# IONIQ6000/av1-go

Hardware: AMD Instinct MI355X
Metric: encoded 4K30 frames/sec (whole node) at fixed QP; PSNR-Y delta vs libaom (higher is better)
Workload: dtype u16

## Files before the change

av1-go_amd/av1stream.py:

```python
import ctypes as C
import os
import subprocess

import numpy as np

_HOST = os.path.join(os.path.dirname(os.path.abspath(__file__)), "host", "libav1mi_host.so")
_lib = None


class ObuFrame(C.Structure):
    _fields_ = [("width", C.c_int32), ("height", C.c_int32), ("bit_depth", C.c_int32), ("frame_type", C.c_int32),
                ("base_q_idx", C.c_int32), ("lf_level", C.c_int32 * 4), ("lf_sharpness", C.c_int32), ("cdef_damping", C.c_int32),
                ("cdef_bits", C.c_int32), ("cdef_y", C.c_uint8 * 8), ("cdef_uv", C.c_uint8 * 8), ("cdef_idx", C.c_void_p),
                ("lr_type", C.c_int32 * 3), ("lr_unit_shift", C.c_int32), ("lr_uv_shift", C.c_int32), ("lr_units", C.c_void_p * 3),
                ("reduced_tx_set", C.c_int32), ("disable_cdf_update", C.c_int32), ("tile_cols_log2", C.c_int32),
                ("tile_rows_log2", C.c_int32), ("y_mode", C.c_void_p), ("angle_y", C.c_void_p), ("uv_mode", C.c_void_p),
                ("angle_uv", C.c_void_p), ("cfl_alpha", C.c_void_p), ("skip", C.c_void_p), ("tx_type", C.c_void_p),
                ("is_inter", C.c_void_p), ("mv", C.c_void_p), ("lev_y", C.c_void_p), ("lev_u", C.c_void_p), ("lev_v", C.c_void_p),
                ("visible_width", C.c_int32), ("visible_height", C.c_int32)]


def lib():
    global _lib
    if _lib is None:
        if not os.path.exists(_HOST):
            subprocess.check_call(["make", "-s", "-C", os.path.dirname(_HOST)])
        _lib = C.CDLL(_HOST)
        _lib.av1mi_obu_write_temporal_unit.restype = C.c_longlong
        _lib.av1mi_obu_write_temporal_unit.argtypes = [C.POINTER(ObuFrame), C.c_int, C.c_int, C.c_void_p, C.c_longlong, C.c_char_p, C.c_int]
        _lib.av1mi_host_opstream_temporal_unit.restype = C.c_longlong
        _lib.av1mi_host_opstream_temporal_unit.argtypes = [C.POINTER(ObuFrame), C.c_int, C.c_void_p, C.c_longlong, C.c_char_p, C.c_int]
    return _lib


_PTR_FIELDS = {"cdef_idx": np.uint8, "y_mode": np.uint8, "angle_y": np.int8, "uv_mode": np.uint8, "angle_uv": np.int8, "cfl_alpha": np.int8,
               "skip": np.uint8, "tx_type": np.uint8, "is_inter": np.uint8, "mv": np.int16, "lev_y": np.int16, "lev_u": np.int16,
               "lev_v": np.int16}


def temporal_unit(width, height, bit_depth, base_q_idx, frame_type=0, with_sequence_header=True, threads=1, lf_level=(0, 0, 0, 0),
                  lf_sharpness=0, cdef_damping=3, cdef_bits=0, cdef_y=(0,), cdef_uv=(0,), lr_type=(0, 0, 0), lr_unit_shift=0, lr_uv_shift=0,
                  lr_units=(None, None, None), reduced_tx_set=0, disable_cdf_update=0, tile_cols_log2=-1, tile_rows_log2=-1, opstream=False,
                  visible=None, key_rows32=0, **arrays):
    f = ObuFrame()
    f.width, f.height, f.bit_depth, f.frame_type, f.base_q_idx = width, height, bit_depth, frame_type, base_q_idx
    if visible is not None:
        f.visible_width, f.visible_height = int(visible[0]), int(visible[1])
    for i in range(4):
        f.lf_level[i] = int(lf_level[i])
    f.lf_sharpness, f.cdef_damping, f.cdef_bits = lf_sharpness, cdef_damping, cdef_bits
    for i, v in enumerate(cdef_y):
        f.cdef_y[i] = int(v)
    for i, v in enumerate(cdef_uv):
        f.cdef_uv[i] = int(v)
    keep = []
    for p in range(3):
        f.lr_type[p] = int(lr_type[p])
        if lr_units[p] is not None:
            a = np.ascontiguousarray(lr_units[p], np.int8)
            keep.append(a)
            f.lr_units[p] = a.ctypes.data
    f.lr_unit_shift, f.lr_uv_shift = lr_unit_shift, lr_uv_shift
    f.reduced_tx_set, f.disable_cdf_update, f.tile_cols_log2, f.tile_rows_log2 = reduced_tx_set, disable_cdf_update, tile_cols_log2, tile_rows_log2
    for k, v in arrays.items():
        if k not in _PTR_FIELDS:
            raise TypeError("unknown field " + k)
        if v is None:
            continue
        a = np.ascontiguousarray(v, _PTR_FIELDS[k])
        keep.append(a)
        setattr(f, k, a.ctypes.data)
    cap = width * height * 4 + (1 << 16)
    out = np.empty(cap, np.uint8)
    err = C.create_string_buffer(256)
    if opstream:
        h = lib()
        h.av1mi_host_opstream_key32_temporal_unit.restype = C.c_longlong
        h.av1mi_host_opstream_key32_temporal_unit.argtypes = [C.POINTER(ObuFrame), C.c_int, C.c_int, C.c_void_p, C.c_longlong, C.c_char_p, C.c_int]
        n = h.av1mi_host_opstream_key32_temporal_unit(C.byref(f), int(key_rows32), int(with_sequence_header), out.ctypes.data, cap, err, 256)
    else:
        n = lib().av1mi_obu_write_temporal_unit(C.byref(f), int(with_sequence_header), threads, out.ctypes.data, cap, err, 256)
    if n < 0:
        raise ValueError("av1 bitstream writer: " + err.value.decode())
    if n > cap:
        raise RuntimeError("temporal unit of %d bytes exceeds the buffer" % n)
    return out[:n].tobytes()


BLOCK_DTYPE = np.dtype([("mi_row", "<u2"), ("mi_col", "<u2"), ("bsize", "u1"), ("skip", "u1"), ("is_inter", "u1"), ("y_mode", "u1"), ("uv_mode", "u1"),
                        ("angle_y", "i1"), ("angle_uv", "i1"), ("cfl_alpha_u", "i1"), ("cfl_alpha_v", "i1"), ("tx_depth", "u1"), ("interp_filter", "u1"),
                        ("reserved", "u1"), ("mv_x", "<i2"), ("mv_y", "<i2"), ("tx_type_off", "<u4"), ("lev_off", "<u4", (3,))])
assert BLOCK_DTYPE.itemsize == 36


class ObuBlocks(C.Structure):
    _fields_ = [("hdr", ObuFrame), ("tx_mode_select", C.c_int32), ("interp_filter", C.c_int32), ("high_precision_mv", C.c_int32), ("partition", C.c_void_p), ("n_partition", C.c_size_t),
                ("blocks", C.c_void_p), ("n_blocks", C.c_size_t), ("tx_type", C.c_void_p), ("levels", C.c_void_p)]


def blocks_temporal_unit(width, height, bit_depth, base_q_idx, partition, blocks, tx_type, levels, frame_type=0, with_sequence_header=True,
                         tx_mode_select=0, interp_filter=0, high_precision_mv=0, reduced_tx_set=0, disable_cdf_update=0, tile_cols_log2=-1,
                         tile_rows_log2=-1, lf_level=(0, 0, 0, 0), lf_sharpness=0, cdef_damping=3, cdef_bits=0, cdef_y=(0,), cdef_uv=(0,), cdef_idx=None,
                         lr_type=(0, 0, 0), lr_units=(None, None, None), lr_unit_shift=0, lr_uv_shift=0):
    d = ObuBlocks()
    f = d.hdr
    f.width, f.height, f.bit_depth, f.frame_type, f.base_q_idx = width, height, bit_depth, frame_type, base_q_idx
    for i in range(4):
        f.lf_level[i] = int(lf_level[i])
    f.lf_sharpness, f.cdef_damping, f.cdef_bits = lf_sharpness, cdef_damping, cdef_bits
    for i, v in enumerate(cdef_y):
        f.cdef_y[i] = int(v)
    for i, v in enumerate(cdef_uv):
        f.cdef_uv[i] = int(v)
    f.reduced_tx_set, f.disable_cdf_update, f.tile_cols_log2, f.tile_rows_log2 = reduced_tx_set, disable_cdf_update, tile_cols_log2, tile_rows_log2
    keep = [np.ascontiguousarray(partition, np.uint8), np.ascontiguousarray(blocks, BLOCK_DTYPE), np.ascontiguousarray(tx_type, np.uint8),
            np.ascontiguousarray(levels, np.int16)]
    if cdef_idx is not None:
        keep.append(np.ascontiguousarray(cdef_idx, np.uint8))
        f.cdef_idx = keep[-1].ctypes.data
    for p in range(3):
        f.lr_type[p] = int(lr_type[p])
        if lr_units[p] is not None:
            keep.append(np.ascontiguousarray(lr_units[p], np.int8))
            f.lr_units[p] = keep[-1].ctypes.data
    f.lr_unit_shift, f.lr_uv_shift = lr_unit_shift, lr_uv_shift
    d.tx_mode_select, d.interp_filter, d.high_precision_mv = int(tx_mode_select), int(interp_filter), int(high_precision_mv)
    d.partition, d.n_partition, d.blocks, d.n_blocks = keep[0].ctypes.data, keep[0].size, keep[1].ctypes.data, keep[1].size
    d.tx_type, d.levels = keep[2].ctypes.data, keep[3].ctypes.data
    cap = width * height * 4 + (1 << 16)
    out = np.empty(cap, np.uint8)
    err = C.create_string_buffer(256)
    L = lib()
    L.av1mi_obu_write_blocks_temporal_unit.restype = C.c_longlong
    L.av1mi_obu_write_blocks_temporal_unit.argtypes = [C.POINTER(ObuBlocks), C.c_int, C.c_void_p, C.c_longlong, C.c_char_p, C.c_int]
    n = L.av1mi_obu_write_blocks_temporal_unit(C.byref(d), int(with_sequence_header), out.ctypes.data, cap, err, 256)
    if n < 0:
        raise ValueError("av1 block writer: " + err.value.decode())
    if n > cap:
        raise RuntimeError("temporal unit of %d bytes exceeds the buffer" % n)
    return out[:n].tobytes()


def assemble_temporal_unit(width, height, bit_depth, base_q_idx, payloads, sizes, with_sequence_header=True, **hdr):
    f = ObuFrame()
    f.width, f.height, f.bit_depth, f.base_q_idx = width, height, bit_depth, base_q_idx
    if hdr.get("visible") is not None:
        f.visible_width, f.visible_height = int(hdr["visible"][0]), int(hdr["visible"][1])
    f.frame_type = hdr.get("frame_type", 0)
    for i in range(4):
        f.lf_level[i] = int(hdr.get("lf_level", (0,) * 4)[i])
    f.lf_sharpness, f.cdef_damping, f.cdef_bits = hdr.get("lf_sharpness", 0), hdr.get("cdef_damping", 3), 0
    f.cdef_y[0], f.cdef_uv[0] = int(hdr.get("cdef_y", (0,))[0]), int(hdr.get("cdef_uv", (0,))[0])
    keep = []
    for p in range(3):
        f.lr_type[p] = int(hdr.get("lr_type", (0, 0, 0))[p])
        u = hdr.get("lr_units", (None,) * 3)[p]
        if u is not None:
            a = np.ascontiguousarray(u, np.int8)
            keep.append(a)
            f.lr_units[p] = a.ctypes.data
    f.lr_unit_shift, f.lr_uv_shift = hdr.get("lr_unit_shift", 0), hdr.get("lr_uv_shift", 0)
    f.tile_cols_log2 = f.tile_rows_log2 = -1
    pay = np.ascontiguousarray(payloads, np.uint8)
    sz = np.ascontiguousarray(sizes, np.uint32)
    cap = int(pay.size) + (1 << 16) + 4 * int(sz.size)
    out = np.empty(cap, np.uint8)
    err = C.create_string_buffer(256)
    L = lib()
    L.av1mi_obu_assemble_temporal_unit.restype = C.c_longlong
    L.av1mi_obu_assemble_temporal_unit.argtypes = [C.POINTER(ObuFrame), C.c_void_p, C.c_void_p, C.c_int, C.c_int, C.c_void_p, C.c_longlong, C.c_char_p, C.c_int]
    n = L.av1mi_obu_assemble_temporal_unit(C.byref(f), pay.ctypes.data, sz.ctypes.data, int(sz.size), int(with_sequence_header), out.ctypes.data, cap, err, 256)
    if n < 0 or n > cap:
        raise ValueError("assemble: " + err.value.decode())
    return out[:n].tobytes()


def session_frame_unit_gpu(width, height, bit_depth, frame, seg, with_sequence_header=None, visible=None):
    p = frame["params"]
    hdr = header_from_params(p, width, height, frame["lr_on"][seg], visible)
    nt = frame["tiles_per_frame"]
    sizes = frame["tile_size"][seg * nt:(seg + 1) * nt]
    start = int(frame["tile_size"][:seg * nt].sum(dtype=np.uint64))
    pay = frame["tile_payload"][start:start + int(sizes.sum(dtype=np.uint64))]
    sh = (p.frame_type == 0) if with_sequence_header is None else with_sequence_header
    return assemble_temporal_unit(width, height, bit_depth, p.base_q_idx, pay, sizes, with_sequence_header=sh, **hdr)


def session_temporal_unit(width, height, bit_depth, raw_frame, seg, with_sequence_header=True, threads=1, visible=None):
    h = lib()
    h.av1mi_session_temporal_unit.restype = C.c_longlong
    h.av1mi_session_temporal_unit.argtypes = [C.c_void_p, C.c_int, C.c_int, C.c_int, C.c_int, C.c_int, C.c_int, C.c_int, C.c_int, C.c_void_p, C.c_longlong,
                                              C.c_char_p, C.c_int]
    cap = width * height * 4 + (1 << 16)
    out = np.empty(cap, np.uint8)
    err = C.create_string_buffer(256)
    vw, vh = visible if visible is not None else (0, 0)
    n = h.av1mi_session_temporal_unit(C.addressof(raw_frame), int(seg), width, height, bit_depth, int(vw), int(vh), int(with_sequence_header), int(threads),
                                      out.ctypes.data, cap, err, 256)
    if n < 0:
        raise ValueError("av1mi_session_temporal_unit: " + err.value.decode())
    return out[:n].tobytes()


def header_from_params(p, width, height, lr_on=None, visible=None):
    ur = lambda n: max(1, (n + p.lr_unit_size // 2) // p.lr_unit_size)
    vw, vh = visible if visible is not None else (width, height)
    uy = np.tile(np.array(list(p.lr_unit_y), np.int8), (ur(vh), ur(vw), 1))
    uc = np.tile(np.array(list(p.lr_unit_uv), np.int8), (ur((vh + 1) // 2), ur((vw + 1) // 2), 1))
    shift = {64: 0, 128: 1, 256: 2}[p.lr_unit_size]
    types = [int(p.lr_unit_y[0]), int(p.lr_unit_uv[0]), int(p.lr_unit_uv[0])]
    if lr_on is not None:
        types = [t if int(k) else 0 for t, k in zip(types, lr_on)]
    return dict(frame_type=p.frame_type, lf_level=tuple(p.lf_level), lf_sharpness=p.lf_sharpness, cdef_damping=p.cdef_damping,
                cdef_y=(p.cdef_y,), cdef_uv=(p.cdef_uv,), lr_type=tuple(types), lr_unit_shift=shift, lr_uv_shift=0, lr_units=(uy, uc, uc),
                **({} if visible is None else {"visible": (int(vw), int(vh))}))


def session_frame_unit(width, height, bit_depth, frame, seg, with_sequence_header=None, threads=1, visible=None):
    p = frame["params"]
    hdr = header_from_params(p, width, height, frame["lr_on"][seg], visible)
    if p.frame_type == 0:
        sym = dict(y_mode=frame["y_mode"][seg], uv_mode=frame["uv_mode"][seg])
    else:
        sym = dict(mv=frame["mv"][seg], skip=frame["skip"][seg])
    sh = (p.frame_type == 0) if with_sequence_header is None else with_sequence_header
    return temporal_unit(width, height, bit_depth, p.base_q_idx, with_sequence_header=sh, threads=threads, lev_y=frame["lev_y"][seg],
                         lev_u=frame["lev_u"][seg], lev_v=frame["lev_v"][seg], **sym, **hdr)
```

av1-go_amd/csrc/av1_entropy_kernels.hip:

```cpp
#include <string.h>
#include <vector>
#include "av1_ops_cdfs.hpp"
#include "av1_ops32.hpp"
#include "av1mi_internal.hpp"

namespace av1mi {
using namespace av1ops;

struct Av1EntLaunch {
  FrameView fv;
  int nframes, sbr_n, sbc_n;
  BlockInfo *info;
  op_t *ops; uint32_t ops_cap;
  uint32_t *grouped; uint32_t grouped_cap;
  uint16_t *slot_total, *slot_base;
  uint16_t *rec;
  uint32_t *nops;
  uint8_t *slots; uint32_t slot_cap;
  uint32_t *tile_size;
  uint64_t *tile_off;
  uint32_t *status;
  uint8_t *out; uint64_t out_cap;
  const uint16_t *cdf_image; int cdf_words;
  SlotTable tab;
  const uint16_t *cdf_image32; SlotTable tab32;
  const uint8_t *lr_on_frame;
  int sb_rows32, band, nslots;
};

__device__ __forceinline__ FrameView frame_view(const Av1EntLaunch &L, int f) {
  FrameView v = L.fv;
  const long nb = (long)v.w8 * v.h8;
  if (v.key) { v.y_mode += nb * f; v.uv_mode += nb * f; }
  else { v.mv += nb * 2 * f; v.skip += nb * f; }
  v.lev_y += nb * 64 * f; v.lev_u += nb * 16 * f; v.lev_v += nb * 16 * f;
  v.info = L.info + nb * f;
  if (L.lr_on_frame) for (int p = 0; p < 3; p++) v.lr_on[p] = v.lr_on[p] && L.lr_on_frame[f * 3 + p];
  return v;
}

__global__ __launch_bounds__(256) void k_av1_info(Av1EntLaunch L) {
  const long nb = (long)L.fv.w8 * L.fv.h8, i = (long)blockIdx.x * 256 + threadIdx.x;
  if (i >= nb * L.nframes) return;
  const int f = (int)(i / nb), b = (int)(i - (long)f * nb);
  const FrameView v = frame_view(L, f);
  BlockInfo o = {};
  block_summary(v, b, &o);
  if (!v.key) inter_mode_decision(v, b / v.w8, b % v.w8, &o);
  L.info[nb * f + b] = o;
}

constexpr int kReplaySlots = (S_MAX + 1) / 2;
struct TokLds {
  union {
    struct { uint8_t cnt[S_MAX * kBlocksPerTile]; alignas(16) uint8_t mag[kBlocksPerTile * kMagBytes]; } p1;
    uint16_t pos[kReplaySlots * kBlocksPerTile];
  };
  uint16_t total[S_MAX], base[S_MAX];
  ScanTables scan;
};

__global__ __launch_bounds__(64) __attribute__((amdgpu_waves_per_eu(2, 8))) void k_av1_tokens(Av1EntLaunch L) {
  const int tiles = L.sbr_n * L.sbc_n, t = blockIdx.x, f = t / tiles, tt = t - f * tiles, sbr = tt / L.sbc_n, sbc = tt - sbr * L.sbc_n;
  if (sbr < L.sb_rows32) return;
  const FrameView v = frame_view(L, f);
  const int zi = threadIdx.x, nslots = v.key ? S_KEY_END : S_INTER_END;
  __shared__ TokLds S;
  {
    uint32_t *m = reinterpret_cast<uint32_t *>(S.p1.cnt);
    for (int i = zi; i < S_MAX * kBlocksPerTile / 4; i += 64) m[i] = 0;
    if (zi == 0) fill_scan_tables(&S.scan);
  }
  __syncthreads();
  uint16_t *rec = L.rec + ((size_t)t * kBlocksPerTile + zi) * kBlockRecords;
  const TokScratch ts = { S.p1.mag + zi * kMagBytes, &S.scan };
  Sink k = { rec, S.p1.cnt, zi, 0, 0, false };
  tok_block(v, k, ts, sbr, sbc, zi);
  int x = k.n;
#pragma unroll
  for (int d = 1; d < 64; d <<= 1) {
    const int y = __shfl_up(x, d, 64);
    if (zi >= d) x += y;
  }
  const int total = __shfl(x, 63, 64), first = x - k.n;
  if ((uint32_t)total > L.ops_cap || __any(k.overflow)) {
    if (zi == 0) { atomicOr(L.status, 1u); L.nops[t] = 0; }
    for (int sl = zi; sl < S_MAX; sl += 64) L.slot_total[(size_t)t * S_MAX + sl] = 0;
    return;
  }
  if (zi == 0) L.nops[t] = (uint32_t)total;
  __syncthreads();
  constexpr int kOwn = (S_MAX + 63) / 64;
  uint32_t c[kOwn][kBlocksPerTile / 4];
#pragma unroll
  for (int q = 0; q < kOwn; q++) {
    const int sl = zi + 64 * q;
    int sum = 0;
#pragma unroll
    for (int w = 0; w < kBlocksPerTile / 4; w++) {
      const uint32_t u = sl < nslots ? reinterpret_cast<const uint32_t *>(S.p1.cnt)[sl * (kBlocksPerTile / 4) + w] : 0u;
      c[q][w] = u;
      sum = (int)__builtin_amdgcn_sad_u8(u, 0u, (unsigned)sum);
    }
    if (sl < S_MAX) S.total[sl] = (uint16_t)sum;
  }
  __syncthreads();
  {
    int mine = 0;
    for (int q = 0; q < 4; q++) { const int sl = 4 * zi + q; if (sl < nslots) mine += (S.total[sl] + kListAlign - 1) & ~(kListAlign - 1); }
    int inc = mine;
#pragma unroll
    for (int d = 1; d < 64; d <<= 1) {
      const int y = __shfl_up(inc, d, 64);
      if (zi >= d) inc += y;
    }
    int run = inc - mine;
    for (int q = 0; q < 4; q++) { const int sl = 4 * zi + q; if (sl < nslots) { S.base[sl] = (uint16_t)run; run += (S.total[sl] + kListAlign - 1) & ~(kListAlign - 1); } }
  }
  __syncthreads();
#pragma unroll
  for (int q = 0; q < kOwn; q++) {
    const int sl = zi + 64 * q;
    if (sl >= S_MAX) continue;
    const bool on = sl < nslots;
    L.slot_total[(size_t)t * S_MAX + sl] = on ? S.total[sl] : (uint16_t)0;
    L.slot_base[(size_t)t * S_MAX + sl] = on ? S.base[sl] : (uint16_t)0;
  }
  op_t *list = L.ops + (size_t)t * L.ops_cap;
  uint32_t *grouped = L.grouped + (size_t)t * L.grouped_cap;
#pragma unroll
  for (int half = 0; half < 2; half++) {
    const int lo = half * kReplaySlots, hi = lo + kReplaySlots;
    if (half) __syncthreads();
#pragma unroll
    for (int q = 0; q < kOwn; q++) {
      const int sl = zi + 64 * q;
      if (sl < lo || sl >= hi || sl >= nslots) continue;
      int run = S.base[sl];
#pragma unroll
      for (int w = 0; w < kBlocksPerTile / 4; w++) {
        const uint32_t u = c[q][w];
        const int p0 = run, p1 = p0 + (int)(u & 0xFF), p2 = p1 + (int)((u >> 8) & 0xFF), p3 = p2 + (int)((u >> 16) & 0xFF);
        run = p3 + (int)(u >> 24);
        uint32_t *d = reinterpret_cast<uint32_t *>(S.pos + (sl - lo) * kBlocksPerTile + 4 * w);
        d[0] = (uint32_t)p0 | ((uint32_t)p1 << 16); d[1] = (uint32_t)p2 | ((uint32_t)p3 << 16);
      }
    }
    __syncthreads();
    __threadfence_block();
    replay_block<kBlocksPerTile>(rec, k.nrec, S.pos, zi, first, list, grouped, lo, hi, half == 0);
  }
}

constexpr int kTiles32 = 16;
static_assert(kBlocks32 * kMag32Bytes >= K_END * kBlocks32 * 2 && kMag32Bytes % 8 == 0, "a tile's counters live where its four magnitude maps were");
__global__ __launch_bounds__(64) void k_av1_tokens32(Av1EntLaunch L, int ntiles_all) {
  __shared__ ScanTables32 scan;
  __shared__ __attribute__((aligned(16))) uint8_t s_mag[64 * kMag32Bytes];
  __shared__ Sum32 s_sum[kTiles32][kBlocks32];
  __shared__ int s_n[kTiles32][kBlocks32], s_nrec[kTiles32][kBlocks32], s_bad[kTiles32];
  const int tiles = L.sbr_n * L.sbc_n, tl = threadIdx.x >> 2, b = threadIdx.x & 3, t = blockIdx.x * kTiles32 + tl;
  bool live = t < ntiles_all;
  int f = 0, sbr = 0, sbc = 0;
  if (live) { f = t / tiles; const int tt = t - f * tiles; sbr = tt / L.sbc_n; sbc = tt - sbr * L.sbc_n; live = sbr < L.sb_rows32; }
  fill_scan_tables32(&scan, (int)threadIdx.x, 64);
  if (b == 0) s_bad[tl] = 0;
  const FrameView v = frame_view(L, live ? f : 0);
  const bool inside = live && !((b & 1) && sbc * 8 + 4 >= v.w8);
  if (inside) block_sums32(v, block_index32(v, sbr, sbc, b), &s_sum[tl][b]);
  __syncthreads();
  uint16_t *rec = L.rec + ((size_t)(live ? t : 0) * kBlocks32 + b) * kBlockRecords32;
  int nrec = 0;
  if (live) { s_n[tl][b] = 0; s_nrec[tl][b] = 0; }
  if (inside) {
    Sink32 k = { rec, nullptr, b, (int)kBlockRecords32, 0, 0, false, 0, 0, 0, 0 };
    const TokScratch32 ts = { s_mag + threadIdx.x * kMag32Bytes, &scan };
    tok_block32(v, k, ts, sbr, sbc, b, s_sum[tl]);
    s_n[tl][b] = k.n; s_nrec[tl][b] = nrec = k.nrec;
    if (k.overflow) atomicOr(&s_bad[tl], 1);
  }
  __syncthreads();
  uint16_t *cnt = reinterpret_cast<uint16_t *>(s_mag + tl * kBlocks32 * kMag32Bytes);
  for (int i = b; i < K_END * kBlocks32; i += kBlocks32) cnt[i] = 0;
  __syncthreads();
  if (live && !count_block32(rec, nrec, cnt, b)) atomicOr(&s_bad[tl], 1);
  __syncthreads();
  if (live && b == 0) {
    uint16_t *total = L.slot_total + (size_t)t * S_MAX, *base = L.slot_base + (size_t)t * S_MAX;
    const int run = place_tile32(cnt, total, base);
    for (int sl = K_END; sl < S_MAX; sl++) { total[sl] = 0; base[sl] = 0; }
    const int n = s_n[tl][0] + s_n[tl][1] + s_n[tl][2] + s_n[tl][3];
    if (s_bad[tl] || (uint32_t)n > L.ops_cap || run > 65535) {
      s_bad[tl] = 1;
      atomicOr(L.status, 1u);
      L.nops[t] = 0;
      for (int sl = 0; sl < K_END; sl++) total[sl] = 0;
    } else {
      L.nops[t] = (uint32_t)n;
    }
  }
  __syncthreads();
  if (!live || s_bad[tl]) return;
  int first = 0;
  for (int q = 0; q < b; q++) first += s_n[tl][q];
  replay_block<kBlocks32>(rec, nrec, cnt, b, first, L.ops + (size_t)t * L.ops_cap, L.grouped + (size_t)t * L.grouped_cap);
}

__global__ __launch_bounds__(64) void k_av1_chains(Av1EntLaunch L, int ntiles_all, int ngroups) {
  const int xcd = blockIdx.x & 7, j = blockIdx.x >> 3, nslots = L.nslots;
  const int g = (j / nslots) * 8 + xcd, sl = j - (j / nslots) * nslots, lane = threadIdx.x, t = g * 64 + lane;
  if (g >= ngroups) return;
  __shared__ __attribute__((aligned(16))) uint16_t s_big[64 * 16];
  const int n = L.tab.nsym[sl], off = L.tab.off[sl];
  int cnt = 0, base = 0;
  bool mine = t < ntiles_all;
  if (mine && L.band) { const int tiles = L.sbr_n * L.sbc_n, sbr = (t % tiles) / L.sbc_n; mine = (sbr < L.sb_rows32) == (L.band == 1); }
  if (mine) { cnt = L.slot_total[(size_t)t * S_MAX + sl]; base = L.slot_base[(size_t)t * S_MAX + sl]; }
  if (!__any(cnt > 0)) return;
  const size_t tt = t < ntiles_all ? (size_t)t : 0;
  op_t *list = L.ops + tt * L.ops_cap;
  const uint32_t *grouped = L.grouped + tt * L.grouped_cap + base;
  if (n <= 4) {
    const uint32_t *iw = reinterpret_cast<const uint32_t *>(L.cdf_image) + (off >> 1);
    uint64_t cdf = (uint64_t)iw[0] | ((uint64_t)iw[1] << 32);
    const uint4 *g4 = reinterpret_cast<const uint4 *>(grouped);
    const uint4 z = make_uint4(0, 0, 0, 0);
    uint4 c0 = cnt > 0 ? g4[0] : z, c1 = cnt > 4 ? g4[1] : z, c2 = cnt > 8 ? g4[2] : z, c3 = cnt > 12 ? g4[3] : z;
    auto four = [&](const uint4 &v, int e) {
      if (e < cnt) list[v.x >> 4] = small_step(cdf, (int)(v.x & 15), n);
      if (e + 1 < cnt) list[v.y >> 4] = small_step(cdf, (int)(v.y & 15), n);
      if (e + 2 < cnt) list[v.z >> 4] = small_step(cdf, (int)(v.z & 15), n);
      if (e + 3 < cnt) list[v.w >> 4] = small_step(cdf, (int)(v.w & 15), n);
    };
#pragma unroll 1
    for (int e = 0; e < cnt; e += 16) {
      const uint4 *nx = g4 + (e >> 2) + 4;
      const uint4 n0 = e + 16 < cnt ? nx[0] : z, n1 = e + 20 < cnt ? nx[1] : z, n2 = e + 24 < cnt ? nx[2] : z, n3 = e + 28 < cnt ? nx[3] : z;
      four(c0, e); four(c1, e + 4); four(c2, e + 8); four(c3, e + 12);
      c0 = n0; c1 = n1; c2 = n2; c3 = n3;
    }
  } else {
    uint16_t *cdf = s_big + lane * 16;
    {
      const uint4 *iw = reinterpret_cast<const uint4 *>(L.cdf_image + off);
      uint4 *d = reinterpret_cast<uint4 *>(cdf);
      d[0] = iw[0];
      d[1] = n > 8 ? iw[1] : make_uint4(0, 0, 0, 0);
    }
#pragma unroll 1
    for (int e = 0; e < cnt; e++) {
      const uint32_t v = grouped[e];
      const int s = (int)(v & 15);
      list[v >> 4] = s >= kSplitHorz ? split_tuple(cdf, s) : big_step(cdf, s, n);
    }
  }
}

constexpr int kRingOps = 64, kLaneWords = kRingOps * 2 + Coder::kStage + 8;

__global__ __launch_bounds__(64) void k_av1_code(Av1EntLaunch L, int ntiles_all) {
  __shared__ __attribute__((aligned(16))) uint16_t s_lane[64 * kLaneWords];
  const int lane = threadIdx.x, t = blockIdx.x * 64 + lane;
  const bool live = t < ntiles_all;
  uint32_t *ring = reinterpret_cast<uint32_t *>(s_lane + lane * kLaneWords);
  Coder c;
  c.init(L.slots + (size_t)(live ? t : 0) * L.slot_cap, (int)L.slot_cap, s_lane + lane * kLaneWords + kRingOps * 2);
  const int n = live ? (int)L.nops[t] : 0;
  const uint4 *ops4 = reinterpret_cast<const uint4 *>(L.ops + (size_t)(live ? t : 0) * L.ops_cap);
  uint4 r0, r1, r2, r3, r4, r5, r6, r7;
  r0 = r1 = r2 = r3 = r4 = r5 = r6 = r7 = make_uint4(0, 0, 0, 0);
  int w = 0;
  bool pend = false;
  auto request = [&]() {
    const uint4 *p = ops4 + (w >> 2);
    if (w < n) r0 = p[0];
    if (w + 4 < n) r1 = p[1];
    if (w + 8 < n) r2 = p[2];
    if (w + 12 < n) r3 = p[3];
    if (w + 16 < n) r4 = p[4];
    if (w + 20 < n) r5 = p[5];
    if (w + 24 < n) r6 = p[6];
    if (w + 28 < n) r7 = p[7];
    pend = w < n;
  };
  auto take = [&]() {
    uint4 *q = reinterpret_cast<uint4 *>(ring + (w & 32));
    q[0] = r0; q[1] = r1; q[2] = r2; q[3] = r3; q[4] = r4; q[5] = r5; q[6] = r6; q[7] = r7;
    w += 32;
  };
  request();
  if (pend) { take(); request(); }
  int i = 0, lit_left = 0;
  uint32_t op = ring[0], op_next = ring[1], op_next2 = ring[2];
  for (;;) {
    if (!__any(lit_left > 0 || i < n)) break;
    if (__any((pend && w - i < 24) || c.ns >= Coder::kStage - 8)) {
      if (pend && w - i <= 32) { take(); request(); }
      c.spill();
    }
#pragma unroll
    for (int q = 0; q < 8; q++) {
      if (lit_left > 0 || i < n) {
        const uint32_t fetched = ring[(i + 3) & (kRingOps - 1)];
        uint32_t tup = op;
        if (lit_left == 0 && (op >> 31)) lit_left = (int)((op >> 27) & 15);
        if (lit_left > 0) {
          lit_left--;
          tup = (op >> lit_left) & 1 ? (1u << 19) | (256u << 9) : (2u << 19) | (512u << 9) | 256u;
        }
        c.encode_tuple(tup);
        if (lit_left == 0) { i++; op = op_next; op_next = op_next2; op_next2 = fetched; }
      }
    }
  }
  if (!live) return;
  int sz = n ? c.finish() : -1;
  if (sz < 0) { if (n) atomicOr(L.status, 2u); sz = 0; }
  L.tile_size[t] = (uint32_t)sz;
}

__global__ __launch_bounds__(1024) void k_av1_scan(Av1EntLaunch L, int ntiles_all) {
  __shared__ uint64_t part[1024];
  const int tid = threadIdx.x, per = (ntiles_all + 1023) / 1024, i0 = tid * per, i1 = min(i0 + per, ntiles_all);
  uint64_t s = 0;
  for (int i = i0; i < i1; i++) s += L.tile_size[i];
  part[tid] = s;
  __syncthreads();
  for (int d = 1; d < 1024; d <<= 1) {
    const uint64_t y = tid >= d ? part[tid - d] : 0;
    __syncthreads();
    part[tid] += y;
    __syncthreads();
  }
  uint64_t run = part[tid] - s;
  for (int i = i0; i < i1; i++) { L.tile_off[i] = run; run += L.tile_size[i]; }
  if (tid == 1023) {
    L.tile_off[ntiles_all] = part[1023];
    if (part[1023] > L.out_cap) atomicOr(L.status, 4u);
  }
}
__global__ __launch_bounds__(64) void k_av1_gather(Av1EntLaunch L) {
  const int t = blockIdx.x;
  const uint32_t n = L.tile_size[t];
  const uint64_t off = L.tile_off[t];
  if (off + n > L.out_cap) return;
  const uint8_t *src = L.slots + (size_t)t * L.slot_cap;
  uint8_t *dst = L.out + off;
  const uint32_t head = min(n, (uint32_t)((16 - (reinterpret_cast<uintptr_t>(dst) & 15)) & 15)), body = (n - head) >> 4, tail0 = head + (body << 4);
  if (threadIdx.x < head) dst[threadIdx.x] = src[threadIdx.x];
  for (uint32_t i = threadIdx.x; i < body; i += 64) {
    uint4 v;
    __builtin_memcpy(&v, src + head + 16 * i, 16);
    *reinterpret_cast<uint4 *>(dst + head + 16 * i) = v;
  }
  if (tail0 + threadIdx.x < n) dst[tail0 + threadIdx.x] = src[tail0 + threadIdx.x];
}

hipError_t launch_av1_front(av1mi_ctx *ctx, const Av1EntLaunch &L, hipStream_t s) {
  const long nb = (long)L.fv.w8 * L.fv.h8 * L.nframes;
  const int ntiles_all = L.sbr_n * L.sbc_n * L.nframes, ngroups = (ntiles_all + 63) / 64;
  ProfToken t = ctx_prof_begin(ctx, AV1MI_K_ENTROPY_TOKENS, s);
  hipLaunchKernelGGL(k_av1_info, dim3((unsigned)((nb + 255) / 256)), dim3(256), 0, s, L);
  if (L.sb_rows32 < L.sbr_n) hipLaunchKernelGGL(k_av1_tokens, dim3((unsigned)ntiles_all), dim3(64), 0, s, L);
  if (L.sb_rows32) hipLaunchKernelGGL(k_av1_tokens32, dim3((unsigned)((ntiles_all + kTiles32 - 1) / kTiles32)), dim3(64), 0, s, L, ntiles_all);
  ctx_prof_end(ctx, t, s);
  t = ctx_prof_begin(ctx, AV1MI_K_ENTROPY_CHAINS, s);
  Av1EntLaunch C = L;
  C.nslots = L.fv.key ? S_KEY_END : S_INTER_END; C.band = L.sb_rows32 ? 2 : 0;
  if (L.sb_rows32 < L.sbr_n) hipLaunchKernelGGL(k_av1_chains, dim3((unsigned)(((ngroups + 7) / 8) * 8 * C.nslots)), dim3(64), 0, s, C, ntiles_all, ngroups);
  if (L.sb_rows32) {
    C.nslots = K_END; C.band = 1; C.tab = L.tab32; C.cdf_image = L.cdf_image32;
    hipLaunchKernelGGL(k_av1_chains, dim3((unsigned)(((ngroups + 7) / 8) * 8 * C.nslots)), dim3(64), 0, s, C, ntiles_all, ngroups);
  }
  ctx_prof_end(ctx, t, s);
  return hipGetLastError();
}
hipError_t launch_av1_back(av1mi_ctx *ctx, const Av1EntLaunch &L, hipStream_t s) {
  const int ntiles_all = L.sbr_n * L.sbc_n * L.nframes;
  ProfToken t = ctx_prof_begin(ctx, AV1MI_K_ENTROPY, s);
  hipLaunchKernelGGL(k_av1_code, dim3((unsigned)((ntiles_all + 63) / 64)), dim3(64), 0, s, L, ntiles_all);
  ctx_prof_end(ctx, t, s);
  t = ctx_prof_begin(ctx, AV1MI_K_ENTROPY_PACK, s);
  hipLaunchKernelGGL(k_av1_scan, dim3(1), dim3(1024), 0, s, L, ntiles_all);
  hipLaunchKernelGGL(k_av1_gather, dim3((unsigned)ntiles_all), dim3(64), 0, s, L);
  ctx_prof_end(ctx, t, s);
  return hipGetLastError();
}

}

struct av1mi_av1ent_state {
  void *info = nullptr, *ops[2] = { nullptr, nullptr }, *nops[2] = { nullptr, nullptr }, *grouped = nullptr, *slot_tb = nullptr, *rec = nullptr, *slots = nullptr, *tile_off = nullptr, *status = nullptr;
  size_t info_b = 0, ops_b[2] = { 0, 0 }, nops_b[2] = { 0, 0 }, grouped_b = 0, slot_tb_b = 0, rec_b = 0, slots_b = 0, off_b = 0;
  hipEvent_t lists_ready[2] = { nullptr, nullptr }, lists_free[2] = { nullptr, nullptr };
  bool free_recorded[2] = { false, false };
  unsigned long jobs = 0;
  av1mi::Av1EntLaunch pending[2];
  uint64_t *pending_total[2] = { nullptr, nullptr };
  bool pending_valid[2] = { false, false };
  size_t last_tiles = 0;
  uint16_t *d_image[2][4] = {};
  uint16_t *d_image32[4] = {};
  av1ops::SlotTable tab32;
  int image_words[2] = { 0, 0 };
  av1ops::SlotTable tab[2];
};

namespace {
int grow(av1mi_ctx *ctx, void **p, size_t *have, size_t need) {
  if (*have >= need) return AV1MI_OK;
  if (*p) (void)hipFree(*p);
  *p = nullptr; *have = 0;
  if (hipMalloc(p, need) != hipSuccess) return av1mi::ctx_fail(ctx, AV1MI_E_NOMEM, "AV1 entropy scratch: hipMalloc(%zu) failed", need);
  *have = need;
  return AV1MI_OK;
}
}

extern "C" {

uint32_t av1mi_av1_entropy_ops_per_tile(void) { return 32768; }
uint32_t av1mi_av1_entropy_slot_bytes(void) { return 16384; }

}

int av1mi::av1_entropy_front(av1mi_ctx *ctx, const av1mi_av1_entropy_job *j, hipStream_t front, int *ticket) {
  if (!ctx || !ticket) return AV1MI_E_INVAL;
  *ticket = -1;
  if (!j) return av1mi::ctx_fail(ctx, AV1MI_E_INVAL, "null job");
  if (hipSetDevice(av1mi::ctx_device(ctx)) != hipSuccess) return av1mi::ctx_fail(ctx, AV1MI_E_DEVICE, "hipSetDevice failed");
  if (j->width <= 0 || j->height <= 0 || (j->width & 7) || (j->height & 7) || j->width > 4096 || j->height > 4096)
    return av1mi::ctx_fail(ctx, AV1MI_E_INVAL, "frame %dx%d must be a multiple of 8, at most 4096x4096", j->width, j->height);
  if (j->nframes < 0 || j->nframes > 4096 || j->base_q_idx < 1 || j->base_q_idx > 255) return av1mi::ctx_fail(ctx, AV1MI_E_INVAL, "bad nframes / base_q_idx");
  const void *need[] = { j->d_lev_y, j->d_lev_u, j->d_lev_v, j->d_out, j->d_tile_size, j->d_total, j->key ? (const void *)j->d_modes_y : (const void *)j->d_mvs,
                         j->key ? (const void *)j->d_modes_uv : (const void *)j->d_skip };
  for (const void *p : need) if (!p) return av1mi::ctx_fail(ctx, AV1MI_E_INVAL, "null device pointer");
  if (j->nframes == 0) return AV1MI_OK;
  av1mi_av1ent_state *st = av1mi::ctx_av1ent(ctx);
  if (!st) return av1mi::ctx_fail(ctx, AV1MI_E_NOMEM, "AV1 entropy state");
  const int key = j->key ? 1 : 0, qcat = av1ops::q_category(j->base_q_idx);
  if (!st->d_image[key][qcat]) {
    av1ops::SlotTable tab;
    const std::vector<uint16_t> img = av1ops::default_slot_image(key != 0, qcat, &tab);
    st->tab[key] = tab; st->image_words[key] = tab.words;
    if (hipMalloc((void **)&st->d_image[key][qcat], img.size() * 2) != hipSuccess ||
        hipMemcpy(st->d_image[key][qcat], img.data(), img.size() * 2, hipMemcpyHostToDevice) != hipSuccess)
      return av1mi::ctx_fail(ctx, AV1MI_E_DEVICE, "uploading the default CDF image failed");
  }
  if (j->key_rows32 && (!key || (j->key_rows32 & 63) || j->key_rows32 > j->height || (j->width & 31)))
    return av1mi::ctx_fail(ctx, AV1MI_E_INVAL, "key_rows32 %d: whole superblock rows of a key frame whose width is a multiple of 32", j->key_rows32);
  if (j->key_rows32 && !st->d_image32[qcat]) {
    const std::vector<uint16_t> img = av1ops::default_slot_image_k32(qcat, &st->tab32);
    if (hipMalloc((void **)&st->d_image32[qcat], img.size() * 2) != hipSuccess ||
        hipMemcpy(st->d_image32[qcat], img.data(), img.size() * 2, hipMemcpyHostToDevice) != hipSuccess)
      return av1mi::ctx_fail(ctx, AV1MI_E_DEVICE, "uploading the default CDF image failed");
  }
  av1mi::Av1EntLaunch L;
  memset(&L, 0, sizeof(L));
  L.sb_rows32 = j->key_rows32 / 64;
  if (j->key_rows32) { L.tab32 = st->tab32; L.cdf_image32 = st->d_image32[qcat]; }
  L.fv.w8 = j->width / 8; L.fv.h8 = j->height / 8; L.fv.key = key;
  L.fv.y_mode = j->d_modes_y; L.fv.uv_mode = j->d_modes_uv; L.fv.mv = j->d_mvs; L.fv.skip = j->d_skip;
  L.fv.lev_y = j->d_lev_y; L.fv.lev_u = j->d_lev_u; L.fv.lev_v = j->d_lev_v;
  for (int p = 0; p < 3; p++) {
    L.fv.lr_on[p] = j->lr_on[p] != 0;
    const int vh = j->visible_height ? j->visible_height : j->height, vw = j->visible_width ? j->visible_width : j->width;
    const int ph = p ? (vh + 1) / 2 : vh, pw = p ? (vw + 1) / 2 : vw;
    L.fv.lr_rows[p] = (ph + 32) / 64 > 1 ? (ph + 32) / 64 : 1; L.fv.lr_cols[p] = (pw + 32) / 64 > 1 ? (pw + 32) / 64 : 1;
  }
  memcpy(L.fv.lr_unit[0], j->lr_unit_y, 8); memcpy(L.fv.lr_unit[1], j->lr_unit_uv, 8);
  L.nframes = j->nframes; L.sbr_n = (L.fv.h8 + 7) / 8; L.sbc_n = (L.fv.w8 + 7) / 8;
  const size_t nb = (size_t)L.fv.w8 * L.fv.h8 * j->nframes, nt = (size_t)L.sbr_n * L.sbc_n * j->nframes;
  L.ops_cap = av1mi_av1_entropy_ops_per_tile(); L.slot_cap = av1mi_av1_entropy_slot_bytes();
  L.grouped_cap = L.ops_cap + av1ops::kListAlign * av1ops::S_MAX;
  const int par = (int)(st->jobs++ & 1);
  st->last_tiles = nt;
  int rc;
  if ((rc = grow(ctx, &st->info, &st->info_b, nb * sizeof(av1ops::BlockInfo))) ||
      (rc = grow(ctx, &st->ops[par], &st->ops_b[par], nt * L.ops_cap * sizeof(av1ops::op_t))) || (rc = grow(ctx, &st->nops[par], &st->nops_b[par], nt * 4)) ||
      (rc = grow(ctx, &st->grouped, &st->grouped_b, nt * L.grouped_cap * sizeof(uint32_t))) ||
      (rc = grow(ctx, &st->slot_tb, &st->slot_tb_b, nt * av1ops::S_MAX * 4)) ||
      (rc = grow(ctx, &st->rec, &st->rec_b, nt * av1ops::kBlocksPerTile * av1ops::kBlockRecords * sizeof(uint16_t))) ||
      (rc = grow(ctx, &st->slots, &st->slots_b, nt * L.slot_cap)) || (rc = grow(ctx, &st->tile_off, &st->off_b, (nt + 1) * 8)))
    return rc;
  L.info = (av1ops::BlockInfo *)st->info; L.ops = (av1ops::op_t *)st->ops[par]; L.nops = (uint32_t *)st->nops[par]; L.grouped = (uint32_t *)st->grouped;
  L.slot_total = (uint16_t *)st->slot_tb; L.slot_base = L.slot_total + nt * av1ops::S_MAX; L.rec = (uint16_t *)st->rec; L.slots = (uint8_t *)st->slots;
  L.tile_off = (uint64_t *)st->tile_off;
  L.tile_size = j->d_tile_size; L.out = j->d_out; L.out_cap = j->out_cap;
  L.status = (uint32_t *)(j->d_total + 1);
  L.cdf_image = st->d_image[key][qcat]; L.cdf_words = st->image_words[key]; L.tab = st->tab[key];
  L.lr_on_frame = j->d_lr_on;
#define E_HIP(call) do { const hipError_t e_ = (call); if (e_ != hipSuccess) return av1mi::ctx_fail(ctx, AV1MI_E_DEVICE, "%s: %s", #call, hipGetErrorString(e_)); } while (0)
  for (hipEvent_t *ev : { &st->lists_ready[par], &st->lists_free[par] }) if (!*ev) E_HIP(hipEventCreateWithFlags(ev, hipEventDisableTiming));
  if (st->free_recorded[par]) E_HIP(hipStreamWaitEvent(front, st->lists_free[par], 0));
  E_HIP(hipMemsetAsync(j->d_total, 0, 16, front));
  E_HIP(av1mi::launch_av1_front(ctx, L, front));
  E_HIP(hipEventRecord(st->lists_ready[par], front));
  st->pending[par] = L; st->pending_total[par] = j->d_total; st->pending_valid[par] = true;
  *ticket = par;
  return AV1MI_OK;
}

int av1mi::av1_entropy_back(av1mi_ctx *ctx, int ticket, hipStream_t back) {
  if (!ctx || ticket < 0 || ticket > 1) return AV1MI_E_INVAL;
  av1mi_av1ent_state *st = av1mi::ctx_av1ent(ctx);
  if (!st || !st->pending_valid[ticket]) return av1mi::ctx_fail(ctx, AV1MI_E_INVAL, "no entropy job pending under this ticket");
  const av1mi::Av1EntLaunch &L = st->pending[ticket];
  const size_t nt = (size_t)L.sbr_n * L.sbc_n * L.nframes;
  E_HIP(hipStreamWaitEvent(back, st->lists_ready[ticket], 0));
  E_HIP(av1mi::launch_av1_back(ctx, L, back));
  E_HIP(hipMemcpyAsync(st->pending_total[ticket], L.tile_off + nt, 8, hipMemcpyDeviceToDevice, back));
  E_HIP(hipEventRecord(st->lists_free[ticket], back)); st->free_recorded[ticket] = true;
  st->pending_valid[ticket] = false;
#undef E_HIP
  return AV1MI_OK;
}

int av1mi::av1_entropy_submit(av1mi_ctx *ctx, const av1mi_av1_entropy_job *j, hipStream_t front, hipStream_t back) {
  int ticket = -1;
  const int rc = av1_entropy_front(ctx, j, front, &ticket);
  if (rc != AV1MI_OK || ticket < 0) return rc;
  return av1_entropy_back(ctx, ticket, back);
}

extern "C" {

int av1mi_av1_entropy_encode_on(av1mi_ctx *ctx, const av1mi_av1_entropy_job *j, void *stream_handle) {
  if (!ctx) return AV1MI_E_INVAL;
  hipStream_t s = stream_handle ? (hipStream_t)stream_handle : av1mi::ctx_stream(ctx);
  return av1mi::av1_entropy_submit(ctx, j, s, s);
}

int av1mi_av1_entropy_encode(av1mi_ctx *ctx, const av1mi_av1_entropy_job *j) { return av1mi_av1_entropy_encode_on(ctx, j, nullptr); }

int av1mi_av1_entropy_last_list_words(av1mi_ctx *ctx, uint64_t *words) {
  if (!ctx || !words) return AV1MI_E_INVAL;
  *words = 0;
  av1mi_av1ent_state *st = av1mi::ctx_av1ent(ctx);
  if (!st || !st->jobs || !st->last_tiles) return AV1MI_OK;
  if (hipSetDevice(av1mi::ctx_device(ctx)) != hipSuccess || hipDeviceSynchronize() != hipSuccess) return av1mi::ctx_fail(ctx, AV1MI_E_DEVICE, "synchronising failed");
  std::vector<uint32_t> n(st->last_tiles);
  if (hipMemcpy(n.data(), st->nops[(st->jobs - 1) & 1], n.size() * 4, hipMemcpyDeviceToHost) != hipSuccess) return av1mi::ctx_fail(ctx, AV1MI_E_DEVICE, "reading the list sizes failed");
  for (uint32_t v : n) *words += v;
  return AV1MI_OK;
}

}

namespace av1mi {
void av1ent_free(av1mi_av1ent_state *st) {
  if (!st) return;
  for (void *p : { st->info, st->ops[0], st->ops[1], st->nops[0], st->nops[1], st->grouped, st->slot_tb, st->rec, st->slots, st->tile_off }) if (p) (void)hipFree(p);
  for (hipEvent_t ev : { st->lists_ready[0], st->lists_ready[1], st->lists_free[0], st->lists_free[1] }) if (ev) (void)hipEventDestroy(ev);
  for (auto &k : st->d_image) for (uint16_t *p : k) if (p) (void)hipFree(p);
  for (uint16_t *p : st->d_image32) if (p) (void)hipFree(p);
  delete st;
}
av1mi_av1ent_state *av1ent_new() { return new (std::nothrow) av1mi_av1ent_state(); }
}
```

av1-go_amd/csrc/av1_ops.hpp:

```cpp
#pragma once
#include <stdint.h>

#if defined(__HIPCC__)
#include <hip/hip_runtime.h>
#define AV1_HD __host__ __device__ inline
#define AV1_UNROLL _Pragma("unroll")
#define AV1_NOUNROLL _Pragma("unroll 1")
#else
#define AV1_HD inline
#define AV1_UNROLL
#define AV1_NOUNROLL
#endif

namespace av1ops {

typedef uint32_t __attribute__((may_alias)) u32a;
typedef uint64_t __attribute__((may_alias)) u64a;

enum Slot : int {
  S_SKIP = 0,
  S_PART8 = S_SKIP + 3,
  S_PART16 = S_PART8 + 1,
  S_PART32 = S_PART16 + 4,
  S_PART64 = S_PART32 + 4,
  S_USE_WIENER = S_PART64 + 4,
  S_TXB_SKIP_Y = S_USE_WIENER + 1,
  S_TXB_SKIP_C = S_TXB_SKIP_Y + 1,
  S_EOB64_Y = S_TXB_SKIP_C + 3,
  S_EOB16_C = S_EOB64_Y + 1,
  S_EOBX_Y = S_EOB16_C + 1,
  S_EOBX_C = S_EOBX_Y + 5,
  S_DC_SIGN_Y = S_EOBX_C + 3,
  S_DC_SIGN_C = S_DC_SIGN_Y + 3,
  S_BASE_EOB_Y = S_DC_SIGN_C + 3,
  S_BASE_EOB_C = S_BASE_EOB_Y + 4,
  S_BASE_Y = S_BASE_EOB_C + 4,
  S_BASE_C = S_BASE_Y + 26,
  S_BR_Y = S_BASE_C + 26,
  S_BR_C = S_BR_Y + 21,
  S_COMMON_END = S_BR_C + 21,
  S_KF_Y_MODE = S_COMMON_END,
  S_UV_MODE = S_KF_Y_MODE + 25,
  S_ANGLE = S_UV_MODE + 13,
  S_INTRA_TX = S_ANGLE + 8,
  S_KEY_END = S_INTRA_TX + 13,
  S_IS_INTER = S_COMMON_END,
  S_SINGLE_REF = S_IS_INTER + 4,
  S_NEW_MV = S_SINGLE_REF + 6,
  S_ZERO_MV = S_NEW_MV + 6,
  S_REF_MV = S_ZERO_MV + 1,
  S_DRL = S_REF_MV + 6,
  S_MV_JOINT = S_DRL + 3,
  S_MV_COMP = S_MV_JOINT + 1,
  S_INTER_TX = S_MV_COMP + 32,
  S_INTER_END = S_INTER_TX + 1,
  S_MAX = S_KEY_END > S_INTER_END ? S_KEY_END : S_INTER_END
};
enum { MVC_CLASS = 0, MVC_CLASS0 = 1, MVC_CLASS0_FR = 2, MVC_SIGN = 4, MVC_BITS = 5, MVC_FR = 15 };

struct BandSlots {
  int use_wiener, kf_y_mode, uv_mode, angle;
  int txb_skip_y, txb_skip_c, eob_y, eob_c, eobx_y, eobx_c, dc_sign_y, dc_sign_c, base_eob_y, base_eob_c, base_y, base_c, br_y, br_c;
  int eob_y_n, eob_c_n;
};
constexpr BandSlots kSlots8 = { S_USE_WIENER, S_KF_Y_MODE, S_UV_MODE, S_ANGLE, S_TXB_SKIP_Y, S_TXB_SKIP_C, S_EOB64_Y, S_EOB16_C, S_EOBX_Y,
                                S_EOBX_C, S_DC_SIGN_Y, S_DC_SIGN_C, S_BASE_EOB_Y, S_BASE_EOB_C, S_BASE_Y, S_BASE_C, S_BR_Y, S_BR_C, 7, 5 };

template <const BandSlots &B> AV1_HD int coeff_nsym(int s) {
  if (s < B.txb_skip_y || s >= B.br_c + 21) return 0;
  if (s == B.eob_y) return B.eob_y_n;
  if (s == B.eob_c) return B.eob_c_n;
  return s < B.base_eob_y ? 2 : s < B.base_y ? 3 : 4;
}
AV1_HD int slot_nsym(int s, bool key) {
  if (const int n = coeff_nsym<kSlots8>(s)) return n;
  if (s < S_PART8) return 2;
  if (s < S_PART16) return 4;
  if (s < S_USE_WIENER) return 10;
  if (s < S_COMMON_END) return 2;
  if (key) {
    if (s < S_UV_MODE) return 13;
    if (s < S_ANGLE) return 14;
    if (s < S_INTRA_TX) return 7;
    return 7;
  }
  if (s < S_MV_JOINT) return 2;
  if (s == S_MV_JOINT) return 4;
  if (s < S_INTER_TX) {
    const int k = (s - S_MV_COMP) & 15;
    return k == MVC_CLASS ? 11 : (k == MVC_CLASS0_FR || k == MVC_CLASS0_FR + 1 || k == MVC_FR) ? 4 : 2;
  }
  return 16;
}
AV1_HD int q_category(int base_q_idx) { return base_q_idx <= 20 ? 0 : base_q_idx <= 60 ? 1 : base_q_idx <= 120 ? 2 : 3; }
AV1_HD int slot_words(int nsym) { return nsym <= 4 ? 4 : nsym <= 8 ? 8 : 16; }

typedef uint32_t op_t;
struct SlotTable { uint16_t off[S_MAX]; uint8_t nsym[(S_MAX + 3) & ~3]; int words; };
AV1_HD op_t op_lit(int n, unsigned v) { return (op_t)(0x80000000u | ((unsigned)n << 27) | (v & 0x7FFu)); }
AV1_HD op_t make_tuple(uint32_t fl, uint32_t fh, int s, int n) { return (op_t)(((unsigned)(n - s) << 19) | ((fl >> 6) << 9) | (fh >> 6)); }
enum { kBlocksPerTile = 64, kSplitHorz = 14, kSplitVert = 15, kListAlign = 4, kBlockRecords = 1024 };

struct Sink {
  uint16_t *rec;
  uint8_t *cnt;
  int zi, nrec, n;
  bool overflow;
  AV1_HD void put(unsigned r) { if (nrec < kBlockRecords) rec[nrec] = (uint16_t)r; else overflow = true; nrec++; n++; }
  AV1_HD void sym(int slot, int s) {
    put(((unsigned)slot << 4) | (unsigned)s);
    uint8_t &c = cnt[slot * kBlocksPerTile + zi];
    if (c == 255) overflow = true; else c++;
  }
  AV1_HD void split(int kind, int slot) { sym(slot, kind ? kSplitVert : kSplitHorz); }
  AV1_HD void lit(unsigned v, int nbits) {
    while (nbits > 11) { nbits -= 11; put(0x8000u | (11u << 11) | ((v >> nbits) & 0x7FFu)); }
    if (nbits > 0) put(0x8000u | ((unsigned)nbits << 11) | (v & ((1u << nbits) - 1u)));
  }
};
AV1_HD int group_positions(const uint8_t *cnt_slot, uint16_t *pos_slot, int base) {
  int run = base;
  for (int b = 0; b < kBlocksPerTile; b++) { const int c = cnt_slot[b]; pos_slot[b] = (uint16_t)run; run += c; }
  return run - base;
}
template <int kBlocks>
AV1_HD void replay_block(const uint16_t *rec, int nrec, uint16_t *pos, int blk, int first, op_t *list, uint32_t *grouped, int slot_lo = 0,
                         int slot_hi = 1 << 16, bool literals = true) {
  int n = first;
  for (int i0 = 0; i0 < nrec; i0 += 8) {
    struct alignas(16) R8 { uint32_t w[4]; } q = *reinterpret_cast<const R8 *>(rec + i0);
    AV1_UNROLL
    for (int j = 0; j < 8; j++, n++) {
      if (i0 + j >= nrec) break;
      const unsigned r = (q.w[j >> 1] >> (16 * (j & 1))) & 0xFFFFu;
      if (r & 0x8000u) { if (literals) list[n] = op_lit((int)((r >> 11) & 15), r & 0x7FFu); }
      else {
        const int sl = (int)(r >> 4);
        if (sl >= slot_lo && sl < slot_hi) { uint16_t &p = pos[(sl - slot_lo) * kBlocks + blk]; grouped[p] = ((uint32_t)n << 4) | (r & 15u); p++; }
      }
    }
  }
}

struct BlockInfo { uint8_t cul[3], dc[3], mode, flags; uint8_t num, drl; int16_t px, py; uint8_t pad[2]; };
struct FrameView {
  int w8, h8;
  int key;
  const uint8_t *y_mode, *uv_mode;
  const int16_t *mv;
  const uint8_t *skip;
  const int16_t *lev_y, *lev_u, *lev_v;
  const BlockInfo *info;
  int lr_on[3];
  int8_t lr_unit[2][8];
  int lr_rows[3], lr_cols[3];
};

AV1_HD int iabs(int v) { return v < 0 ? -v : v; }
AV1_HD int imin(int a, int b) { return a < b ? a : b; }
AV1_HD int imax(int a, int b) { return a > b ? a : b; }
AV1_HD int ilog2(unsigned v) { return 31 - __builtin_clz(v | 1u); }
AV1_HD unsigned morton8(unsigned x, unsigned y) {
  unsigned m = 0;
  for (int i = 0; i < 3; i++) m |= ((x >> i) & 1u) << (2 * i) | ((y >> i) & 1u) << (2 * i + 1);
  return m;
}
AV1_HD void demorton8(unsigned k, int *bx, int *by) {
  int x = 0, y = 0;
  for (int i = 0; i < 3; i++) { x |= ((k >> (2 * i)) & 1) << i; y |= ((k >> (2 * i + 1)) & 1) << i; }
  *bx = x; *by = y;
}

AV1_HD void block_summary(const FrameView &f, int b, BlockInfo *o) {
  const int16_t *p[3] = { f.lev_y + (long)b * 64, f.lev_u + (long)b * 16, f.lev_v + (long)b * 16 };
  const bool skip = !f.key && f.skip[b];
  for (int pl = 0; pl < 3; pl++) {
    int cul = 0;
    const int n = pl ? 16 : 64;
    for (int i = 0; i < n; i++) cul += iabs(p[pl][i]);
    o->cul[pl] = skip ? 0 : (uint8_t)imin(cul, 63);
    o->dc[pl] = skip ? 0 : (uint8_t)(p[pl][0] < 0 ? 1 : p[pl][0] > 0 ? 2 : 0);
  }
}

struct MvCand { int16_t x, y; int weight; };
struct MvStack { MvCand st[8]; int num, new_ctx, ref_ctx; };

AV1_HD void mv_stack(const FrameView &f, int r8, int c8, bool use_flags, MvStack *S) {
  const int r0 = r8 & ~7, c0 = c8 & ~7, r1 = imin(r0 + 8, f.h8), c1 = imin(c0 + 8, f.w8);
  int num = 0, new_count = 0;
  bool found = false;
  MvCand *st = S->st;
  auto add = [&](int r, int c, bool count_new) {
    if (r < r0 || r >= r1 || c < c0 || c >= c1) return;
    const int nb = r * f.w8 + c;
    const int16_t mx = f.mv[2 * nb], my = f.mv[2 * nb + 1];
    if (count_new && use_flags && (f.info[nb].flags & 1)) new_count++;
    found = true;
    int i = 0;
    for (; i < num; i++) if (st[i].x == mx && st[i].y == my) break;
    if (i < num) st[i].weight += 4;
    else if (num < 8) { st[num].x = mx; st[num].y = my; st[num].weight = 4; num++; }
  };
  add(r8 - 1, c8, true);
  const bool above0 = found; found = false;
  add(r8, c8 - 1, true);
  const bool left0 = found; found = false;
  {
    const int tr = r8 - 1, tc = c8 + 1;
    if (tr >= r0 && tc < c1 && morton8(tc & 7, tr & 7) < morton8(c8 & 7, r8 & 7)) add(tr, tc, true);
  }
  bool above = above0 || found; found = false;
  const int close = (above ? 1 : 0) + (left0 ? 1 : 0);
  const int num_nearest = num, num_new = new_count;
  for (int i = 0; i < num_nearest; i++) st[i].weight += 640;
  add(r8 - 1, c8 - 1, false);
  above = above || found; found = false;
  bool left = left0;
  add(r8 - 2, c8, false); above = above || found; found = false;
  add(r8, c8 - 2, false); left = left || found; found = false;
  add(r8 - 3, c8, false); above = above || found; found = false;
  add(r8, c8 - 3, false); left = left || found; found = false;
  const int total = (above ? 1 : 0) + (left ? 1 : 0);
  for (int pass = 0; pass < 2; pass++) {
    const int a = pass ? num_nearest : 0, bnd = pass ? num : num_nearest;
    for (int len = bnd; len > a;) {
      int nr = a;
      for (int i = a + 1; i < len; i++)
        if (st[i - 1].weight < st[i].weight) { const MvCand t = st[i - 1]; st[i - 1] = st[i]; st[i] = t; nr = i; }
      len = nr;
    }
  }
  if (close == 0) { S->new_ctx = imin(total, 1); S->ref_ctx = total; }
  else if (close == 1) { S->new_ctx = 3 - imin(num_new, 1); S->ref_ctx = 2 + total; }
  else { S->new_ctx = 5 - imin(num_new, 1); S->ref_ctx = 5; }
  const int mi_r = r8 * 2, mi_c = c8 * 2, border = 128 + 2 * 4 * 8;
  const int top = -(mi_r * 32) - border, bottom = (f.h8 * 2 - 2 - mi_r) * 32 + border;
  const int lft = -(mi_c * 32) - border, right = (f.w8 * 2 - 2 - mi_c) * 32 + border;
  for (int i = 0; i < num; i++) {
    st[i].y = (int16_t)imin(imax(st[i].y, top), bottom);
    st[i].x = (int16_t)imin(imax(st[i].x, lft), right);
  }
  for (int i = num; i < 2; i++) { st[i].x = st[i].y = 0; st[i].weight = 0; }
  S->num = num;
}
AV1_HD void inter_mode_decision(const FrameView &f, int r8, int c8, BlockInfo *o) {
  MvStack S;
  mv_stack(f, r8, c8, false, &S);
  const int b = r8 * f.w8 + c8, mx = f.mv[2 * b], my = f.mv[2 * b + 1];
  int mode = 3, ref_idx = 0;
  if (S.st[0].x == mx && S.st[0].y == my) mode = 0;
  else {
    for (int i = 1; i < imax(S.num, 2) && i < 4; i++)
      if (S.st[i].x == mx && S.st[i].y == my) { mode = 1; ref_idx = i; break; }
    if (mode == 3 && mx == 0 && my == 0) mode = 2;
  }
  if (mode == 3) {
    const int nsel = imin(S.num, 3);
    long best = -1;
    for (int i = 0; i < imax(nsel, 1); i++) {
      const long c = iabs(mx - S.st[i].x) + iabs(my - S.st[i].y);
      if (best < 0 || c < best) { best = c; ref_idx = i; }
    }
  }
  o->mode = (uint8_t)(mode | (ref_idx << 2));
  o->flags = (uint8_t)(mode == 3);
  o->num = (uint8_t)S.num;
  int drl = 0;
  for (int i = 0; i < 4; i++) if (i < imax(S.num, 2) && S.st[i].weight >= 640) drl |= 1 << i;
  o->drl = (uint8_t)drl;
  const int pred = S.num <= 1 ? 0 : ref_idx;
  o->px = S.st[pred].x; o->py = S.st[pred].y;
}

template <class K> AV1_HD void tok_subexp(K &k, int num_syms, int kk, int v) {
  int i = 0, mk = 0;
  for (;;) {
    const int b2 = i ? kk + i - 1 : kk, a = 1 << b2;
    if (num_syms <= mk + 3 * a) {
      const int n = num_syms - mk, x = v - mk, w = ilog2((unsigned)n) + 1, m = (1 << w) - n;
      if (x < m) k.lit((unsigned)x, w - 1);
      else { k.lit((unsigned)((x + m) >> 1), w - 1); k.lit((unsigned)((x + m) & 1), 1); }
      return;
    }
    const int more = v >= mk + a;
    k.lit((unsigned)more, 1);
    if (!more) { k.lit((unsigned)(v - mk), b2); return; }
    i++; mk += a;
  }
}
AV1_HD int tok_recenter(int r, int v) { return v > 2 * r ? v : v >= r ? 2 * (v - r) : 2 * (r - v) - 1; }
template <class K> AV1_HD void tok_signed_subexp_ref(K &k, int v, int low, int high, int kk, int r) {
  const int mx = high - low;
  v -= low; r -= low;
  tok_subexp(k, mx, kk, (r << 1) <= mx ? tok_recenter(r, v) : tok_recenter(mx - 1 - r, mx - 1 - v));
}
template <const BandSlots &B, class K> AV1_HD void tok_lr(const FrameView &f, K &k, int sbr, int sbc) {
  const int mi_r = sbr * 16, mi_c = sbc * 16;
  for (int p = 0; p < 3; p++) {
    if (!f.lr_on[p]) continue;
    const int ss = p ? 1 : 0, us = 64;
    const int row0 = (mi_r * (4 >> ss) + us - 1) / us, row1 = imin(((mi_r + 16) * (4 >> ss) + us - 1) / us, f.lr_rows[p]);
    const int col0 = (mi_c * (4 >> ss) + us - 1) / us, col1 = imin(((mi_c + 16) * (4 >> ss) + us - 1) / us, f.lr_cols[p]);
    const int8_t *u = f.lr_unit[p ? 1 : 0];
    for (int ur = row0; ur < row1; ur++)
      for (int uc = col0; uc < col1; uc++) {
        k.sym(B.use_wiener, u[0] == 1);
        if (u[0] != 1) continue;
        const int kmin[3] = { -5, -23, -17 }, kmax[3] = { 10, 8, 46 }, kk[3] = { 1, 2, 3 }, mid[3] = { 3, -7, 15 };
        for (int pass = 0; pass < 2; pass++)
          for (int j = p ? 1 : 0; j < 3; j++) tok_signed_subexp_ref(k, u[1 + pass * 3 + j], kmin[j], kmax[j] + 1, kk[j], mid[j]);
      }
  }
}
template <const BandSlots &B, class K> AV1_HD void tok_kf_modes(K &k, int ym, int uvm, int above, int left) {
  static const uint8_t kCtx[13] = { 0, 1, 2, 3, 4, 4, 4, 4, 3, 0, 1, 2, 0 };
  k.sym(B.kf_y_mode + kCtx[above] * 5 + kCtx[left], ym);
  if (ym >= 1 && ym <= 8) k.sym(B.angle + ym - 1, 3);
  k.sym(B.uv_mode + ym, uvm);
  if (uvm >= 1 && uvm <= 8) k.sym(B.angle + uvm - 1, 3);
}
AV1_HD void tok_partition_prefix(const FrameView &f, Sink &k, int sbr, int sbc, int bx, int by) {
  const int mi_rows = f.h8 * 2, mi_cols = f.w8 * 2;
  for (int bsize = 64; bsize >= 16; bsize >>= 1) {
    const int n8 = bsize >> 3;
    if ((bx & (n8 - 1)) || (by & (n8 - 1))) continue;
    const int r = (sbr * 8 + by) * 2, c = (sbc * 8 + bx) * 2, half = bsize >> 3;
    const bool has_rows = r + half < mi_rows, has_cols = c + half < mi_cols;
    const bool au = by > 0, al = bx > 0;
    const int slot = (bsize == 16 ? S_PART16 : bsize == 32 ? S_PART32 : S_PART64) + (al ? 2 : 0) + (au ? 1 : 0);
    if (has_rows && has_cols) k.sym(slot, 3);
    else if (has_cols) k.split(0, slot);
    else if (has_rows) k.split(1, slot);
  }
  k.sym(S_PART8, 0);
}

struct ScanTables { uint8_t s4[16], s8[64], i4[16], i8[64]; };
AV1_HD void fill_scan_tables(ScanTables *t) {
  for (int N = 4; N <= 8; N += 4) {
    uint8_t *o = N == 4 ? t->s4 : t->s8;
    int k = 0;
    for (int d = 0; d < 2 * N - 1; d++)
      for (int i = 0; i <= d; i++) {
        const int r = (d & 1) ? i : d - i, c = d - r;
        if (r < N && c < N) o[k++] = (uint8_t)(r * N + c);
      }
    uint8_t *inv = N == 4 ? t->i4 : t->i8;
    for (int i = 0; i < N * N; i++) inv[o[i]] = (uint8_t)i;
  }
}
enum { kMagStride = 10, kMagBytes = 100 };
struct TokScratch { uint8_t *mag; const ScanTables *scan; };

template <int N, bool kBytes = (N <= 8)> struct MagMap;
template <int N> struct MagMap<N, true> {
  enum { LG = N == 4 ? 2 : 3, MS = kMagStride };
  uint8_t *mag;
  const uint8_t *scan, *iscan;
  AV1_HD MagMap(const TokScratch &ts) : mag(ts.mag), scan(N == 4 ? ts.scan->s4 : ts.scan->s8), iscan(N == 4 ? ts.scan->i4 : ts.scan->i8) {}
  AV1_HD int load(const int16_t *lev) {
    for (int i = 0; i < (N + 2) * MS / 4; i++) reinterpret_cast<u32a *>(mag)[i] = 0;
    int eob = 0;
    for (int r = 0; r < N * N / 8; r++) {
      struct alignas(16) L8 { int16_t v[8]; } q = *reinterpret_cast<const L8 *>(lev + 8 * r);
      for (int j = 0; j < 8; j++) {
        const int pos = 8 * r + j, v = q.v[j], a = iabs(v);
        if (v) eob = imax(eob, iscan[pos] + 1);
        mag[(pos >> LG) * MS + (pos & (N - 1))] = (uint8_t)((a > 15 ? 15 : a) | (v < 0 ? 128 : 0));
      }
    }
    return eob;
  }
  AV1_HD int pos(int c) const { return scan[c]; }
  AV1_HD int at(int i) const { return mag[i] & 15; }
  AV1_HD int neg(int p) const { return mag[(p >> LG) * MS + (p & (N - 1))] >> 7; }
};

template <int N, const BandSlots &B, class K, class TS>
AV1_HD void tok_coeffs(K &k, const TS &ts, bool chroma, const int16_t *lev, int above_cul, int above_dc, int left_cul, int left_dc, int tx_slot,
                       int tx_sym) {
  MagMap<N> M(ts);
  const int nc = N * N, LG = M.LG, MS = M.MS;
  const int eob = M.load(lev);
  k.sym(chroma ? B.txb_skip_c + ((above_cul | above_dc) != 0) + ((left_cul | left_dc) != 0) : B.txb_skip_y, eob == 0);
  if (!eob) return;
  if (tx_slot >= 0) k.sym(tx_slot, tx_sym);
  const int eob_pt = eob < 3 ? eob : ilog2((unsigned)(eob - 1)) + 2;
  k.sym(chroma ? B.eob_c : B.eob_y, eob_pt - 1);
  if (eob_pt >= 3) {
    const int off = eob - ((1 << (eob_pt - 2)) + 1), shift = eob_pt - 3;
    k.sym((chroma ? B.eobx_c : B.eobx_y) + eob_pt - 3, (off >> shift) & 1);
    if (shift > 0) k.lit((unsigned)(off & ((1 << shift) - 1)), shift);
  }
  const int base_eob = chroma ? B.base_eob_c : B.base_eob_y, base = chroma ? B.base_c : B.base_y, br = chroma ? B.br_c : B.br_y;
  for (int c = eob - 1; c >= 0; c--) {
    const int pos = M.pos(c), row = pos >> LG, col = pos & (N - 1), at = row * MS + col;
    const int m0 = M.at(at), m1 = M.at(at + 1), m2 = M.at(at + 2), mb = M.at(at + MS), md = M.at(at + MS + 1), mbb = M.at(at + 2 * MS);
    int a = m0;
    if (a == 15) a = iabs(lev[pos]);
    if (c == eob - 1) {
      k.sym(base_eob + (c == 0 ? 0 : c <= nc / 8 ? 1 : c <= nc / 4 ? 2 : 3), imin(a, 3) - 1);
    } else {
      const int mm = imin(m1, 3) + imin(mb, 3) + imin(md, 3) + imin(m2, 3) + imin(mbb, 3);
      int bctx = imin((mm + 1) >> 1, 4);
      if (pos == 0) bctx = 0;
      else bctx += row + col < 2 ? 1 : row + col < 4 ? 6 : 21;
      k.sym(base + bctx, imin(a, 3));
    }
    if (a > 2) {
      int mm = m1 + mb + md;
      mm = imin((mm + 1) >> 1, 6);
      const int rctx = pos == 0 ? mm : (row < 2 && col < 2) ? mm + 7 : mm + 14;
      int rem = a - 3;
      for (int i = 0; i < 4; i++) {
        const int q = imin(rem, 3);
        k.sym(br + rctx, q);
        rem -= q;
        if (q < 3) break;
      }
    }
  }
  for (int c = 0; c < eob; c++) {
    const int pos = M.pos(c), m = M.at((pos >> LG) * MS + (pos & (N - 1)));
    if (!m) continue;
    const int neg = M.neg(pos);
    if (c == 0) {
      const int sg = (above_dc == 2) - (above_dc == 1) + (left_dc == 2) - (left_dc == 1);
      k.sym((chroma ? B.dc_sign_c : B.dc_sign_y) + (sg < 0 ? 1 : sg > 0 ? 2 : 0), neg);
    } else {
      k.lit((unsigned)neg, 1);
    }
    if (m == 15) {
      const int a = iabs(lev[pos]);
      if (a > 14) {
        const unsigned x = (unsigned)(a - 14);
        const int len = ilog2(x) + 1;
        k.lit(0, len - 1);
        k.lit(x, len);
      }
    }
  }
}

AV1_HD void tok_mv_comp(Sink &k, int comp, int diff) {
  const int base = S_MV_COMP + comp * 16;
  k.sym(base + MVC_SIGN, diff < 0);
  const int off = iabs(diff) - 1, cls = (off >> 3) < 2 ? 0 : ilog2((unsigned)(off >> 3));
  k.sym(base + MVC_CLASS, cls);
  if (cls == 0) {
    k.sym(base + MVC_CLASS0, off >> 3);
    k.sym(base + MVC_CLASS0_FR + (off >> 3), (off >> 1) & 3);
  } else {
    const int o = off - (2 << (cls + 2)), d = o >> 3;
    for (int i = 0; i < cls; i++) k.sym(base + MVC_BITS + i, (d >> i) & 1);
    k.sym(base + MVC_FR, (o >> 1) & 3);
  }
}

AV1_HD void tok_block(const FrameView &f, Sink &k, const TokScratch &ts, int sbr, int sbc, int zi) {
  int bx, by;
  demorton8((unsigned)zi, &bx, &by);
  const int r8 = sbr * 8 + by, c8 = sbc * 8 + bx;
  if (r8 >= f.h8 || c8 >= f.w8) return;
  if (zi == 0) tok_lr<kSlots8>(f, k, sbr, sbc);
  tok_partition_prefix(f, k, sbr, sbc, bx, by);
  const int b = r8 * f.w8 + c8;
  const bool au = by > 0, al = bx > 0;
  const BlockInfo zero = {};
  const BlockInfo ia = au ? f.info[b - f.w8] : zero, il = al ? f.info[b - 1] : zero;
  const int skip = f.key ? 0 : f.skip[b];
  k.sym(S_SKIP + (au && !f.key ? f.skip[b - f.w8] : 0) + (al && !f.key ? f.skip[b - 1] : 0), skip);
  int ym = 0;
  if (f.key) {
    ym = f.y_mode[b];
    tok_kf_modes<kSlots8>(k, ym, f.uv_mode[b], au ? f.y_mode[b - f.w8] : 0, al ? f.y_mode[b - 1] : 0);
  } else {
    k.sym(S_IS_INTER + 0, 1);
    const int rctx = (au || al) ? 1 : 0;
    k.sym(S_SINGLE_REF + rctx * 3 + 0, 0);
    k.sym(S_SINGLE_REF + rctx * 3 + 1, 0);
    k.sym(S_SINGLE_REF + rctx * 3 + 2, 0);
    const BlockInfo me = f.info[b];
    const int mode = me.mode & 3, ref_idx = me.mode >> 2, num = me.num;
    const int mx = f.mv[2 * b], my = f.mv[2 * b + 1];
    const int close = (au ? 1 : 0) + (al ? 1 : 0);
    int num_new = (au ? ia.flags & 1 : 0) + (al ? il.flags & 1 : 0);
    if (au && bx < 7 && c8 + 1 < f.w8 && morton8((unsigned)bx + 1, (unsigned)by - 1) < morton8((unsigned)bx, (unsigned)by)) num_new += f.info[b - f.w8 + 1].flags & 1;
    const int new_ctx = close == 0 ? 0 : close == 1 ? 3 - imin(num_new, 1) : 5 - imin(num_new, 1);
    const int ref_ctx = close == 0 ? 0 : close == 1 ? 3 : 5;
    k.sym(S_NEW_MV + new_ctx, mode != 3);
    if (mode != 3) {
      k.sym(S_ZERO_MV, mode != 2);
      if (mode != 2) k.sym(S_REF_MV + ref_ctx, mode == 1);
    }
    auto drl_ctx = [&](int i) {
      const bool a = (me.drl >> i) & 1, c = (me.drl >> (i + 1)) & 1;
      return a && c ? 0 : a ? 1 : !c ? 2 : 0;
    };
    if (mode == 3) {
      for (int i = 0; i < 2; i++)
        if (num > i + 1) {
          k.sym(S_DRL + drl_ctx(i), ref_idx != i);
          if (ref_idx == i) break;
        }
      const int dx = mx - me.px, dy = my - me.py;
      k.sym(S_MV_JOINT, (dx ? 1 : 0) + (dy ? 2 : 0));
      if (dy) tok_mv_comp(k, 0, dy);
      if (dx) tok_mv_comp(k, 1, dx);
    } else if (mode == 1) {
      for (int i = 1; i < 3; i++)
        if (num > i + 1) {
          k.sym(S_DRL + drl_ctx(i), ref_idx != i);
          if (ref_idx == i) break;
        }
    }
  }
  if (skip) return;
  tok_coeffs<8, kSlots8>(k, ts, false, f.lev_y + (long)b * 64, ia.cul[0], ia.dc[0], il.cul[0], il.dc[0], f.key ? S_INTRA_TX + ym : S_INTER_TX, f.key ? 1 : 7);
  AV1_NOUNROLL
  for (int p = 1; p < 3; p++)
    tok_coeffs<4, kSlots8>(k, ts, true, (p == 1 ? f.lev_u : f.lev_v) + (long)b * 16, ia.cul[p], ia.dc[p], il.cul[p], il.dc[p], -1, 0);
}

template <class F> AV1_HD void build_slot_table(int n, F nsym, SlotTable *t) {
  int o = 0;
  for (int s = 0; s < S_MAX; s++) {
    if (s < n) {
      t->nsym[s] = (uint8_t)nsym(s);
      const int w = slot_words(t->nsym[s]), al = w < 8 ? 4 : 8;
      o = (o + al - 1) & ~(al - 1);
      t->off[s] = (uint16_t)o;
      o += w;
    } else { t->nsym[s] = 2; t->off[s] = 0; }
  }
  t->words = (o + 7) & ~7;
}
AV1_HD void build_slot_table(bool key, SlotTable *t) { build_slot_table(key ? S_KEY_END : S_INTER_END, [key](int s) { return slot_nsym(s, key); }, t); }

#ifdef AV1_CODER_STATS
static long long coder_stat_carries = 0;
#endif
struct Coder {
  enum { kStage = 32 };
  uint64_t low;
  uint32_t rng;
  int nb;
  uint8_t *out;
  uint16_t *stage;
  int pos, cap, ns;
  bool overflow;
  AV1_HD void init(uint8_t *o, int c, uint16_t *st) { low = 0; rng = 0x8000; nb = -1; out = o; stage = st; pos = 0; cap = c; ns = 0; overflow = false; }
  AV1_HD void carry_back() {
    for (int k = ns; k-- > 0;) { const uint16_t v = (uint16_t)(stage[k] + 1); stage[k] = v; if (v) return; }
    for (int i = pos; i-- > 0;) if (++out[i] != 0) return;
  }
  AV1_HD bool stage_full() const { return ns >= kStage - 1; }
  AV1_HD void spill() {
    if (pos + 2 * ns > cap) { overflow = true; pos += 2 * ns; ns = 0; return; }
    for (int k = 0; k < ns; k++) { const uint32_t v = stage[k]; *reinterpret_cast<uint16_t *>(out + pos + 2 * k) = (uint16_t)((v >> 8) | (v << 8)); }
    pos += 2 * ns; ns = 0;
  }
  AV1_HD void flush16() {
    nb -= 16;
    const uint32_t w = (uint32_t)(low >> (16 + nb));
    if ((w >> 16) && !overflow) {
#ifdef AV1_CODER_STATS
      coder_stat_carries++;
#endif
      carry_back();
    }
    stage[ns++] = (uint16_t)w;
    low &= ((uint64_t)1 << (16 + nb)) - 1;
  }
  AV1_HD void encode(uint32_t fl, uint32_t fh, int s, int n) {
    const uint32_t r = rng, v = (((r >> 8) * (fh >> 6)) >> 1) + 4u * (uint32_t)(n - 1 - s);
    const uint32_t u = fl < 32768u ? (((r >> 8) * (fl >> 6)) >> 1) + 4u * (uint32_t)(n - s) : r;
    low += r - u;
    const uint32_t nr = u - v;
    const int d = 15 - ilog2(nr);
    rng = nr << d; low <<= d; nb += d;
    if (nb >= 32) flush16();
  }
  AV1_HD void encode_tuple(op_t t) {
    const uint32_t fl6 = (t >> 9) & 1023u, fh6 = t & 511u, dl = (t >> 19) & 31u;
    const uint32_t r = rng, v = (((r >> 8) * fh6) >> 1) + 4u * (dl - 1u);
    const uint32_t u = fl6 < 512u ? (((r >> 8) * fl6) >> 1) + 4u * dl : r;
    low += r - u;
    const uint32_t nr = u - v;
    const int d = 15 - ilog2(nr);
    rng = nr << d; low <<= d; nb += d;
    if (nb >= 32) flush16();
  }
  AV1_HD void bit(int b) { encode(b ? 16384u : 32768u, b ? 0u : 16384u, b, 2); }
  AV1_HD int finish() {
    uint64_t e = ((low + 0x3FFF) & ~(uint64_t)0x3FFF) | 0x4000;
    if (nb >= 0 && (e >> (16 + nb))) { if (!overflow) carry_back(); e &= ((uint64_t)1 << (16 + nb)) - 1; }
    spill();
    int top = 15 + nb;
    while (top >= 14) {
      uint8_t byte = 0;
      for (int q = 7; q >= 0 && top >= 14; q--, top--) byte |= (uint8_t)(((e >> top) & 1) << q);
      if (pos < cap) out[pos] = byte; else overflow = true;
      pos++;
    }
    return overflow ? -1 : pos;
  }
};

AV1_HD uint32_t adapt(uint32_t x, bool below, int rate) {
  const uint32_t m = 0u - (uint32_t)below, d = ((x ^ m) + (m & 32769u)) >> rate;
  return x - ((d ^ m) - m);
}

AV1_HD op_t small_step(uint64_t &w, int s, int n) {
  const uint32_t x0 = (uint32_t)w & 0xFFFFu, x1 = (uint32_t)w >> 16, x2 = (uint32_t)(w >> 32) & 0xFFFFu, cnt = (uint32_t)(w >> 48);
  const uint32_t fl = s == 0 ? 32768u : s == 1 ? x0 : s == 2 ? x1 : x2;
  const uint32_t fh = s == n - 1 ? 0u : s == 0 ? x0 : s == 1 ? x1 : x2;
  const int rate = 3 + (cnt > 15) + (cnt > 31) + (n >= 4 ? 2 : 1);
  const uint32_t y0 = adapt(x0, 0 < s, rate), y1 = adapt(x1, 1 < s, rate), y2 = adapt(x2, 2 < s, rate), ncnt = cnt + (cnt < 32);
  w = (uint64_t)(y0 | (y1 << 16)) | ((uint64_t)(y2 | (ncnt << 16)) << 32);
  return make_tuple(fl, fh, s, n);
}

AV1_HD op_t big_step(uint16_t *v, int s, int n) {
  const int nd = n > 8 ? 8 : 4;
  u32a *d = reinterpret_cast<u32a *>(v);
  uint32_t w[8];
  AV1_UNROLL
  for (int k = 0; k < 8; k++) w[k] = k < nd ? d[k] : 0u;
  const uint32_t fl = s ? v[s - 1] : 32768u, fh = s == n - 1 ? 0u : v[s];
  const uint32_t cnt = (nd == 8 ? w[7] : w[3]) >> 16;
  const int rate = 3 + (cnt > 15) + (cnt > 31) + 2;
  AV1_UNROLL
  for (int k = 0; k < 8; k++) {
    if (k >= nd) continue;
    uint32_t lo = adapt(w[k] & 0xFFFFu, 2 * k < s, rate), hi = adapt(w[k] >> 16, 2 * k + 1 < s, rate);
    if (k == nd - 1) hi = cnt + (cnt < 32);
    d[k] = lo | (hi << 16);
  }
  return make_tuple(fl, fh, s, n);
}

AV1_HD op_t split_tuple(const uint16_t *p, int kind) {
  const uint32_t p1 = p[0] - p[1], p2 = p[1] - p[2], p3 = p[2] - p[3], p4 = p[3] - p[4], p5 = p[4] - p[5], p6 = p[5] - p[6], p7 = p[6] - p[7],
                 p8 = p[7] - p[8], p9 = p[8];
  return make_tuple(kind == kSplitHorz ? p2 + p3 + p4 + p6 + p7 + p9 : p1 + p3 + p4 + p5 + p6 + p8, 0, 1, 2);
}

AV1_HD void run_chain(const uint16_t *init, int n, const uint32_t *g, int cnt, op_t *list) {
  if (n <= 4) {
    uint64_t w = (uint64_t)init[0] | ((uint64_t)init[1] << 16) | ((uint64_t)init[2] << 32) | ((uint64_t)init[3] << 48);
    for (int k = 0; k < cnt; k++) list[g[k] >> 4] = small_step(w, (int)(g[k] & 15), n);
    return;
  }
  alignas(16) uint16_t v[16];
  for (int i = 0; i < 16; i++) v[i] = i < slot_words(n) ? init[i] : 0;
  for (int k = 0; k < cnt; k++) {
    const int s = (int)(g[k] & 15);
    list[g[k] >> 4] = s >= kSplitHorz ? split_tuple(v, s) : big_step(v, s, n);
  }
}

AV1_HD void code_word(Coder &c, op_t e) {
  if (e >> 31) { for (int i = (int)((e >> 27) & 15) - 1; i >= 0; i--) { c.bit((e >> i) & 1); if (c.stage_full()) c.spill(); } }
  else { c.encode_tuple(e); if (c.stage_full()) c.spill(); }
}

}
```

av1-go_amd/host/av1_bitstream.hpp:

```cpp
#pragma once
#include <cstddef>
#include <cstdint>
#include <string>
#include <vector>

#include "../../include/av1mi_host.h"

namespace av1mi_host {
namespace av1 {

struct SequenceParams {
  int width = 0, height = 0, bit_depth = 8;
  bool operator==(const SequenceParams &o) const { return width == o.width && height == o.height && bit_depth == o.bit_depth; }
};

inline int visible_width(const av1mi_obu_frame &f) { return f.visible_width ? f.visible_width : f.width; }
inline int visible_height(const av1mi_obu_frame &f) { return f.visible_height ? f.visible_height : f.height; }
inline SequenceParams sequence_params(const av1mi_obu_frame &f) {
  SequenceParams sp; sp.width = visible_width(f); sp.height = visible_height(f); sp.bit_depth = f.bit_depth;
  return sp;
}
std::vector<uint8_t> temporal_delimiter_obu();
std::vector<uint8_t> sequence_header_obu(const SequenceParams &sp);
bool frame_obu(const av1mi_obu_frame &f, int threads, std::vector<uint8_t> *out, std::string *err);
bool frame_obu_from_tiles(const av1mi_obu_frame &f, const uint8_t *payloads, const uint32_t *sizes, int ntiles, std::vector<uint8_t> *out,
                          std::string *err);
std::vector<uint8_t> range_code_raw(const uint32_t *fl, const uint32_t *fh, const uint8_t *sym, const uint8_t *nsym, size_t count);
bool opstream_supported(const av1mi_obu_frame &f, std::string *why);
bool opstream_tiles(const av1mi_obu_frame &f, std::vector<std::vector<uint8_t>> *tiles, std::string *err, int key_rows32 = 0);
bool blocks_temporal_unit(const av1mi_obu_blocks &d, bool with_sequence_header, std::vector<uint8_t> *out, std::string *err, int threads = 1,
                          const size_t (*tile_start)[2] = nullptr);
bool temporal_unit(const av1mi_obu_frame &f, bool with_sequence_header, int threads, std::vector<uint8_t> *out, std::string *err);

}
}
```

av1-go_amd/host/av1_opstream.cpp:

```cpp
#include <algorithm>
#include <cstdio>
#include <cstdlib>
#include <cstring>
#include <string>
#include <vector>
#include "../csrc/av1_ops_cdfs.hpp"
#include "av1_bitstream.hpp"

namespace av1mi_host {
namespace av1 {

bool opstream_supported(const av1mi_obu_frame &f, std::string *why) {
  auto no = [&](const char *m) { if (why) *why = m; return false; };
  if (f.cdef_bits || f.reduced_tx_set || f.disable_cdf_update) return no("cdef_bits / reduced_tx_set / disable_cdf_update must be 0");
  if (f.tile_cols_log2 >= 0 || f.tile_rows_log2 >= 0) return no("one superblock per tile only");
  if (f.angle_y || f.angle_uv || f.cfl_alpha || f.tx_type || f.is_inter) return no("angle deltas, chroma from luma, transform types and intra blocks in inter frames are host-writer only");
  if (f.frame_type == 0 && f.skip) return no("key frames are coded with skip = 0");
  for (int p = 0; p < 3; p++) if (f.lr_type[p] > 1) return no("Wiener restoration only");
  if (f.lr_unit_shift || f.lr_uv_shift) return no("64x64 restoration units only");
  return true;
}

namespace {
template <int kBlocks>
bool code_tile(const uint16_t *rec, int block_records, const int *nrec, const int *first, uint16_t *pos, int nslots, const uint16_t *total,
               const uint16_t *base, int run, const av1ops::SlotTable &tab, const uint16_t *image, std::vector<uint8_t> *out, std::string *err) {
  using namespace av1ops;
  if (run > 65535) { if (err) *err = "tile too large for 16-bit entry positions"; return false; }
  const int nops = first[kBlocks];
  std::vector<op_t> list((size_t)nops, 0);
  std::vector<uint32_t> grouped((size_t)run, 0);
  for (int b = 0; b < kBlocks; b++) replay_block<kBlocks>(rec + (size_t)b * block_records, nrec[b], pos, b, first[b], list.data(), grouped.data());
  for (int sl = 0; sl < nslots; sl++)
    if (total[sl]) run_chain(&image[tab.off[sl]], tab.nsym[sl], &grouped[(size_t)base[sl]], total[sl], list.data());
  out->resize((size_t)nops * 2 + 64);
  Coder c;
  uint16_t stage[Coder::kStage];
  c.init(out->data(), (int)out->size(), stage);
  for (int i = 0; i < nops; i++) code_word(c, list[(size_t)i]);
  const int n = c.finish();
  if (n < 0) { if (err) *err = "tile payload overflow"; return false; }
  out->resize((size_t)n);
  return true;
}
}

bool opstream_tiles(const av1mi_obu_frame &f, std::vector<std::vector<uint8_t>> *tiles, std::string *err, int key_rows32) {
  using namespace av1ops;
  if (!opstream_supported(f, err)) return false;
  if (key_rows32 && (f.frame_type != 0 || (key_rows32 & 63) || key_rows32 > f.height || (f.width & 31))) { if (err) *err = "bad 32x32 band"; return false; }
  FrameView v;
  memset(&v, 0, sizeof(v));
  v.w8 = f.width / 8; v.h8 = f.height / 8; v.key = f.frame_type == 0;
  v.y_mode = f.y_mode; v.uv_mode = f.uv_mode; v.mv = f.mv; v.skip = f.skip; v.lev_y = f.lev_y; v.lev_u = f.lev_u; v.lev_v = f.lev_v;
  std::vector<uint8_t> zskip;
  if (!v.key && !v.skip) { zskip.assign((size_t)v.w8 * v.h8, 0); v.skip = zskip.data(); }
  for (int p = 0; p < 3; p++) {
    v.lr_on[p] = f.lr_type[p] == 1;
    const int ph = p ? (visible_height(f) + 1) >> 1 : visible_height(f), pw = p ? (visible_width(f) + 1) >> 1 : visible_width(f);
    v.lr_rows[p] = std::max((ph + 32) / 64, 1); v.lr_cols[p] = std::max((pw + 32) / 64, 1);
  }
  for (int p = 0; p < 3; p++) {
    if (!v.lr_on[p]) continue;
    const int8_t *u = f.lr_units[p];
    const size_t n = (size_t)v.lr_rows[p] * v.lr_cols[p];
    for (size_t i = 1; i < n; i++) if (memcmp(u, u + i * 8, 8)) { if (err) *err = "restoration units must be uniform per plane"; return false; }
    if (p == 2 && v.lr_on[1] && memcmp(u, f.lr_units[1], 8)) { if (err) *err = "U and V restoration units must be equal"; return false; }
    memcpy(v.lr_unit[p ? 1 : 0], u, 8);
  }
  const size_t nb = (size_t)v.w8 * v.h8;
  std::vector<BlockInfo> info(nb);
  v.info = info.data();
  for (size_t b = 0; b < nb; b++) { memset(&info[b], 0, sizeof(BlockInfo)); block_summary(v, (int)b, &info[b]); }
  if (!v.key) for (int r = 0; r < v.h8; r++) for (int c = 0; c < v.w8; c++) inter_mode_decision(v, r, c, &info[(size_t)r * v.w8 + c]);
  const int qcat = q_category(f.base_q_idx);
  SlotTable tab;
  const std::vector<uint16_t> image = default_slot_image(v.key != 0, qcat, &tab);
  const int sbr_n = (v.h8 + 7) / 8, sbc_n = (v.w8 + 7) / 8;
  tiles->assign((size_t)sbr_n * sbc_n, {});
  const int nslots = v.key ? S_KEY_END : S_INTER_END;
  std::vector<uint8_t> cnt((size_t)S_MAX * kBlocksPerTile);
  std::vector<uint16_t> pos((size_t)S_MAX * kBlocksPerTile), rec((size_t)kBlocksPerTile * kBlockRecords);
  ScanTables scan;
  fill_scan_tables(&scan);
  alignas(16) uint8_t mag[kMagBytes];
  const TokScratch ts = { mag, &scan };
  const bool stats = getenv("AV1MI_TOK_STATS") != nullptr;
  int st_rec = 0, st_cnt = 0, st_ops = 0, st_over = 0; long st_ops_sum = 0;
  SlotTable tab32;
  const std::vector<uint16_t> image32 = key_rows32 ? default_slot_image_k32(qcat, &tab32) : std::vector<uint16_t>();
  std::vector<uint16_t> rec32(key_rows32 ? (size_t)kBlocksPerTile * kBlockRecords : 0), cnt32((size_t)K_END * kBlocks32);
  std::vector<ScanTables32> scan32(key_rows32 ? 1 : 0);
  if (key_rows32) fill_scan_tables32(scan32.data());
  alignas(16) uint8_t mag32[kMag32Bytes];
  for (int sbr = 0; sbr < sbr_n; sbr++)
    for (int sbc = 0; sbc < sbc_n; sbc++) {
      if (sbr * 64 < key_rows32) {
        std::fill(cnt32.begin(), cnt32.end(), 0);
        const TokScratch32 ts32 = { mag32, scan32.data() };
        Sum32 sums[kBlocks32];
        const bool half = sbc * 8 + 4 >= v.w8;
        for (int b = 0; b < kBlocks32; b++) if (!(half && (b & 1))) block_sums32(v, block_index32(v, sbr, sbc, b), &sums[b]);
        int nrec[kBlocks32], first[kBlocks32 + 1];
        first[0] = 0;
        for (int b = 0; b < kBlocks32; b++) {
          Sink32 k = { &rec32[(size_t)b * kBlockRecords32], cnt32.data(), b, (int)kBlockRecords32, 0, 0, false, 0, 0, 0, 0 };
          tok_block32(v, k, ts32, sbr, sbc, b, sums);
          if (k.overflow) { if (err) *err = "a block exceeds the tokenizer's record area"; return false; }
          nrec[b] = k.nrec; first[b + 1] = first[b] + k.n;
        }
        for (int b = 0; b < kBlocks32; b++)
          if (!count_block32(&rec32[(size_t)b * kBlockRecords32], nrec[b], cnt32.data(), b)) { if (err) *err = "too many symbols of one slot in a block"; return false; }
        uint16_t base[K_END], total[K_END];
        const int run = place_tile32(cnt32.data(), total, base);
        if (!code_tile<kBlocks32>(rec32.data(), kBlockRecords32, nrec, first, cnt32.data(), K_END, total, base, run, tab32, image32.data(),
                                  &(*tiles)[(size_t)sbr * sbc_n + sbc], err))
          return false;
        continue;
      }
      std::fill(cnt.begin(), cnt.end(), 0);
      int first[kBlocksPerTile + 1], nrec[kBlocksPerTile];
      first[0] = 0;
      bool over = false;
      for (int zi = 0; zi < kBlocksPerTile; zi++) {
        Sink k = { &rec[(size_t)zi * kBlockRecords], cnt.data(), zi, 0, 0, false };
        tok_block(v, k, ts, sbr, sbc, zi);
        if (k.overflow && !stats) { if (err) *err = "a block exceeds the tokenizer's record area"; return false; }
        over |= k.overflow;
        nrec[zi] = k.nrec;
        first[zi + 1] = first[zi] + k.n;
        if (k.nrec > st_rec) st_rec = k.nrec;
      }
      if (stats) {
        for (uint8_t c : cnt) if (c > st_cnt) st_cnt = c;
        if (first[kBlocksPerTile] > st_ops) st_ops = first[kBlocksPerTile];
        st_ops_sum += first[kBlocksPerTile];
        if (over) { st_over++; continue; }
      }
      uint16_t base[S_MAX], total[S_MAX];
      int run = 0;
      for (int sl = 0; sl < nslots; sl++) {
        const int n = group_positions(&cnt[(size_t)sl * kBlocksPerTile], &pos[(size_t)sl * kBlocksPerTile], run);
        base[sl] = (uint16_t)run; total[sl] = (uint16_t)n;
        run = (run + n + kListAlign - 1) & ~(kListAlign - 1);
      }
      if (!code_tile<kBlocksPerTile>(rec.data(), kBlockRecords, nrec, first, pos.data(), nslots, total, base, run, tab, image.data(),
                                     &(*tiles)[(size_t)sbr * sbc_n + sbc], err))
        return false;
    }
  if (stats)
    fprintf(stderr, "[av1mi tok stats] %d tiles: records per block <= %d (capacity %d), symbols of a slot in a block <= %d (255), list words per tile <= %d, mean %.0f; %d tiles over a block capacity\n",
            sbr_n * sbc_n, st_rec, (int)kBlockRecords, st_cnt, st_ops, (double)st_ops_sum / (sbr_n * sbc_n), st_over);
  return true;
}

}
}
```

av1-go_amd/host/capi_host.cpp:

```cpp
#include <cstring>
#include "daemon.hpp"
#include "av1_bitstream.hpp"
#include "mux.hpp"
#include "y4m.hpp"
#include "backend.hpp"

using namespace av1mi_host;

extern "C" {
int av1mi_host_determine_quality(int height) { return DetermineQuality(height); }
int av1mi_host_check_size_gate(long long orig, long long neu, double ratio) { return CheckSizeGate(orig, neu, ratio) ? 1 : 0; }
int av1mi_host_transcode_args(const char *in, const char *out, int has_video, int index, int height, int webrip, char *buf, int cap) {
  ProbeResult pr; pr.has_video_stream = has_video != 0; pr.VideoStream.Index = index; pr.VideoStream.Height = height;
  std::vector<std::string> a; std::string err;
  const bool ok = TranscodeArgs("ffmpeg", in, out, pr, webrip != 0, &a, &err);
  std::string j;
  if (ok) for (size_t i = 0; i < a.size(); i++) j += (i ? "\n" : "") + a[i]; else j = err;
  strncpy(buf, j.c_str(), cap - 1); buf[cap - 1] = 0;
  return ok ? (int)a.size() : -1;
}
long long av1mi_host_y4m_scan(const char *path, int group, unsigned long long *sum, int *seekable, int *geometry, char *err, int cap) {
  Y4mSource y;
  std::string e;
  auto fail = [&]() { strncpy(err, e.c_str(), cap - 1); err[cap - 1] = 0; return -1LL; };
  if (!y.open(path, &e)) return fail();
  const int cw = (y.w + 7) & ~7, ch = (y.h + 7) & ~7;
  const size_t bps = y.bd == 8 ? 1 : 2;
  std::vector<unsigned char> Y((size_t)cw * ch * bps), U((size_t)cw * ch * bps / 4), V((size_t)cw * ch * bps / 4);
  unsigned long long acc = 1469598103934665603ull;
  long long total = 0;
  for (long first = 0;; first += group) {
    const long n = y.prepare(first, group, &e);
    if (n < 0) return fail();
    if (n == 0) break;
    for (long i = 0; i < n; i++) {
      if (!y.read(i, cw, ch, Y.data(), U.data(), V.data())) { e = "read failed"; return fail(); }
      for (const auto *pl : { &Y, &U, &V }) for (unsigned char b : *pl) acc = (acc ^ b) * 1099511628211ull;
    }
    total += n;
  }
  *sum = acc; *seekable = y.seekable() ? 1 : 0;
  geometry[0] = y.w; geometry[1] = y.h; geometry[2] = y.bd; geometry[3] = y.fps_n; geometry[4] = y.fps_d;
  return total;
}
int av1mi_host_y4m_sar(const char *path, int *sar) {
  Y4mSource y;
  std::string e;
  if (!y.open(path, &e)) return -1;
  sar[0] = y.sar_n; sar[1] = y.sar_d;
  return 0;
}
int av1mi_host_scale_target(int iw, int ih, int sar_n, int sar_d, const char *chain, int *w, int *h) {
  std::string e;
  bool square = false;
  return ScaleTarget(iw, ih, sar_n, sar_d, chain ? chain : "", w, h, &square, &e) ? 0 : -1;
}
int av1mi_host_mux_selftest(const char *out_path, int width, int height, int bit_depth, int fps_n, int fps_d, const unsigned char *units,
                            const long long *off, int n_units, int gop, const char *sides, char *err, int cap) {
  std::string e;
  auto fail = [&]() { strncpy(err, e.c_str(), cap - 1); err[cap - 1] = 0; return -1; };
  StreamSink sink;
  for (std::string rest = sides ? sides : ""; !rest.empty();) {
    const size_t nl = rest.find('\n');
    const std::string one = rest.substr(0, nl);
    rest = nl == std::string::npos ? "" : rest.substr(nl + 1);
    if (!one.empty() && !sink.add_side_file(one, &e)) return fail();
  }
  av1::SequenceParams sp;
  sp.width = width; sp.height = height; sp.bit_depth = bit_depth;
  if (!sink.open(out_path, sp, fps_n, fps_d, &e)) return fail();
  for (int i = 0; i < n_units; i++) {
    const std::vector<uint8_t> tu(units + off[i], units + off[i + 1]);
    if (!sink.write(tu, i % gop == 0, &e)) { sink.abort(); return fail(); }
  }
  if (!sink.close(&e)) return fail();
  return 0;
}
int av1mi_run_transcode(int argc, const char *const *argv, char *err, size_t errcap) {
  std::vector<std::string> a;
  for (int i = 0; i < argc; i++) a.push_back(argv[i] ? argv[i] : "");
  const RunResult rr = RunTranscode("av1mi", a);
  if (err && errcap) { strncpy(err, rr.err.c_str(), errcap - 1); err[errcap - 1] = 0; }
  return rr.exitCode;
}
int av1mi_host_run_transcode(const char *joined, char *buf, int cap) {
  std::vector<std::string> a; std::string s = joined; size_t p = 0, q;
  while ((q = s.find('\n', p)) != std::string::npos) { a.push_back(s.substr(p, q - p)); p = q + 1; }
  a.push_back(s.substr(p));
  const RunResult rr = RunTranscode("av1mi", a);
  strncpy(buf, rr.err.c_str(), cap - 1); buf[cap - 1] = 0;
  return rr.exitCode;
}
int av1mi_host_process_job(const char *source, long long orig_size, double ratio, const char *state_dir, int wait_s, int replace_source,
                           char *status, char *reason, int cap) {
  Job job; job.ID = "test"; job.SourcePath = source; job.OriginalSize = orig_size;
  TranscodeConfig cfg; cfg.MaxSizeRatio = ratio; cfg.JobStateDir = state_dir ? state_dir : ""; cfg.StableWaitSeconds = wait_s;
  cfg.ReplaceSource = replace_source != 0;
  ProbeResult pr; pr.HasVideo = true; pr.has_video_stream = true; pr.VideoStream.Height = 720;
  const std::string e = ProcessJob(&job, "av1mi", pr, cfg);
  strncpy(status, job.Status.c_str(), cap - 1); status[cap - 1] = 0;
  strncpy(reason, job.Reason.c_str(), cap - 1); reason[cap - 1] = 0;
  return e.empty() ? 0 : 1;
}
long long av1mi_obu_write_temporal_unit(const av1mi_obu_frame *f, int with_sequence_header, int threads, uint8_t *out, long long cap,
                                        char *err, int errcap) {
  std::vector<uint8_t> b; std::string e;
  if (!av1::temporal_unit(*f, with_sequence_header != 0, threads, &b, &e)) {
    if (err && errcap > 0) { strncpy(err, e.c_str(), errcap - 1); err[errcap - 1] = 0; }
    return -1;
  }
  if ((long long)b.size() <= cap && out) memcpy(out, b.data(), b.size());
  return (long long)b.size();
}
long long av1mi_session_temporal_unit(const av1mi_gop_frame *fr, int seg, int width, int height, int bit_depth, int visible_width, int visible_height,
                                      int with_sequence_header, int threads, uint8_t *out, long long cap, char *err, int errcap) {
  std::vector<uint8_t> b; std::string e;
  if (!fr || seg < 0 || seg >= fr->segments) e = "bad batch / segment";
  else if (SessionTemporalUnit(*fr, seg, width, height, bit_depth, visible_width, visible_height, with_sequence_header != 0, threads, &b, &e)) {
    if ((long long)b.size() <= cap && out) memcpy(out, b.data(), b.size());
    return (long long)b.size();
  }
  if (err && errcap > 0) { strncpy(err, e.c_str(), errcap - 1); err[errcap - 1] = 0; }
  return -1;
}
long long av1mi_obu_write_blocks_temporal_unit(const av1mi_obu_blocks *f, int with_sequence_header, uint8_t *out, long long cap, char *err, int errcap) {
  std::vector<uint8_t> b; std::string e;
  if (!f || !av1::blocks_temporal_unit(*f, with_sequence_header != 0, &b, &e)) {
    if (err && errcap > 0) { strncpy(err, f ? e.c_str() : "null description", errcap - 1); err[errcap - 1] = 0; }
    return -1;
  }
  if ((long long)b.size() <= cap && out) memcpy(out, b.data(), b.size());
  return (long long)b.size();
}
long long av1mi_obu_assemble_temporal_unit(const av1mi_obu_frame *f, const uint8_t *payloads, const uint32_t *sizes, int ntiles,
                                           int with_sequence_header, uint8_t *out, long long cap, char *err, int errcap) {
  std::vector<uint8_t> fr; std::string e;
  if (!av1::frame_obu_from_tiles(*f, payloads, sizes, ntiles, &fr, &e)) {
    if (err && errcap > 0) { strncpy(err, e.c_str(), errcap - 1); err[errcap - 1] = 0; }
    return -1;
  }
  std::vector<uint8_t> b = av1::temporal_delimiter_obu();
  if (with_sequence_header) {
    const av1::SequenceParams sp = av1::sequence_params(*f);
    const std::vector<uint8_t> sh = av1::sequence_header_obu(sp);
    b.insert(b.end(), sh.begin(), sh.end());
  }
  b.insert(b.end(), fr.begin(), fr.end());
  if ((long long)b.size() <= cap && out) memcpy(out, b.data(), b.size());
  return (long long)b.size();
}
long long av1mi_host_opstream_key32_temporal_unit(const av1mi_obu_frame *f, int key_rows32, int with_sequence_header, uint8_t *out, long long cap, char *err,
                                                  int errcap) {
  std::vector<std::vector<uint8_t>> tiles; std::string e;
  auto fail = [&](long long code) { if (err && errcap > 0) { strncpy(err, e.c_str(), errcap - 1); err[errcap - 1] = 0; } return code; };
  if (!av1::opstream_supported(*f, &e)) return fail(-2);
  if (!av1::opstream_tiles(*f, &tiles, &e, key_rows32)) return fail(-1);
  std::vector<uint8_t> cat; std::vector<uint32_t> sizes;
  for (auto &t : tiles) { sizes.push_back((uint32_t)t.size()); cat.insert(cat.end(), t.begin(), t.end()); }
  std::vector<uint8_t> fr;
  if (!av1::frame_obu_from_tiles(*f, cat.data(), sizes.data(), (int)sizes.size(), &fr, &e)) return fail(-1);
  std::vector<uint8_t> b = av1::temporal_delimiter_obu();
  if (with_sequence_header) {
    const av1::SequenceParams sp = av1::sequence_params(*f);
    const std::vector<uint8_t> sh = av1::sequence_header_obu(sp);
    b.insert(b.end(), sh.begin(), sh.end());
  }
  b.insert(b.end(), fr.begin(), fr.end());
  if ((long long)b.size() <= cap && out) memcpy(out, b.data(), b.size());
  return (long long)b.size();
}
long long av1mi_host_opstream_temporal_unit(const av1mi_obu_frame *f, int with_sequence_header, uint8_t *out, long long cap, char *err, int errcap) {
  return av1mi_host_opstream_key32_temporal_unit(f, 0, with_sequence_header, out, cap, err, errcap);
}
int av1mi_host_job_json(const char *id, const char *source, const char *status, const char *reason, long long orig, long long neu, char *buf, int cap) {
  Job j; j.ID = id; j.SourcePath = source; j.Status = status; j.Reason = reason; j.OriginalSize = orig; j.NewSize = neu; j.CreatedAt = "2026-01-02T03:04:05Z";
  const std::string s = JobToJSON(j);
  strncpy(buf, s.c_str(), cap - 1); buf[cap - 1] = 0;
  return (int)s.size();
}
double av1mi_host_gpu_usage(int device, const char *sysfs_root) { return GetGPUUsage(device, sysfs_root ? sysfs_root : "/sys"); }
int av1mi_host_mux_units(const char *path, int w, int h, int bd, int fps_n, int fps_d, const uint8_t *data, const long long *sizes,
                         const uint8_t *keys, int n) {
  StreamSink sink; std::string err;
  av1::SequenceParams sp; sp.width = w; sp.height = h; sp.bit_depth = bd;
  if (!sink.open(path, sp, fps_n, fps_d, &err)) return 1;
  for (int i = 0; i < n; i++) {
    std::vector<uint8_t> tu(data, data + sizes[i]);
    data += sizes[i];
    if (!sink.write(tu, keys[i] != 0, &err)) { sink.abort(); return 2; }
  }
  return sink.close(&err) ? 0 : 3;
}
int av1mi_host_mux_units_display(const char *path, int w, int h, int bd, int fps_n, int fps_d, const uint8_t *data, const long long *sizes,
                                 const uint8_t *keys, int n, int display_w, int display_h) {
  StreamSink sink; std::string err;
  av1::SequenceParams sp; sp.width = w; sp.height = h; sp.bit_depth = bd;
  if (display_w || display_h) sink.set_display_size(display_w, display_h);
  if (!sink.open(path, sp, fps_n, fps_d, &err)) return 1;
  for (int i = 0; i < n; i++) {
    std::vector<uint8_t> tu(data, data + sizes[i]);
    data += sizes[i];
    if (!sink.write(tu, keys[i] != 0, &err)) { sink.abort(); return 2; }
  }
  return sink.close(&err) ? 0 : 3;
}
int av1mi_host_job_pool(const char *sources, int workers, int ngpus, double ratio, const char *state_dir, char *buf, int cap) {
  std::vector<Job> jobs; std::string s = sources; size_t p = 0, q;
  auto add = [&](const std::string &path) {
    Job j; j.ID = "pool" + std::to_string(jobs.size()); j.SourcePath = path;
    FILE *f = fopen(path.c_str(), "rb");
    if (f) { fseek(f, 0, SEEK_END); j.OriginalSize = ftell(f); fclose(f); }
    jobs.push_back(j);
  };
  while ((q = s.find('\n', p)) != std::string::npos) { add(s.substr(p, q - p)); p = q + 1; }
  add(s.substr(p));
  TranscodeConfig cfg; cfg.MaxSizeRatio = ratio; cfg.JobStateDir = state_dir ? state_dir : ""; cfg.StableWaitSeconds = 0;
  ProbeResult pr; pr.HasVideo = true; pr.has_video_stream = true; pr.VideoStream.Height = 720;
  std::vector<std::string> errs;
  const PoolStats ps = RunJobPool(&jobs, workers, ngpus, pr, cfg, &errs);
  std::string out;
  for (size_t i = 0; i < jobs.size(); i++) out += (i ? "\n" : "") + jobs[i].Status + (errs[i].empty() ? "" : ": " + errs[i]);
  strncpy(buf, out.c_str(), cap - 1); buf[cap - 1] = 0;
  return ps.succeeded;
}
}
```

Baseline: 2814.

## Write chain results in place into grouped buffer and resolve refs at coding time

Chain kernels now overwrite the grouped symbol buffer with coded tuples using vectorized uint4 stores, instead of scattering each result to its position in the per-tile op list. The op list instead holds reference words that the coding kernel resolves with a gather from the grouped buffer while filling its ring. The grouped buffer is double-buffered per parity, and the XCD-interleaved block mapping in the chains launch is dropped. This trades random scattered writes for an extra dependent gather in the coder's refill path. A host-side tile trace API is also added for debugging.

```diff
diff --git a/av1-go_amd/av1stream.py b/av1-go_amd/av1stream.py
--- a/av1-go_amd/av1stream.py
+++ b/av1-go_amd/av1stream.py
@@ -41,7 +41,7 @@
 def temporal_unit(width, height, bit_depth, base_q_idx, frame_type=0, with_sequence_header=True, threads=1, lf_level=(0, 0, 0, 0),
                   lf_sharpness=0, cdef_damping=3, cdef_bits=0, cdef_y=(0,), cdef_uv=(0,), lr_type=(0, 0, 0), lr_unit_shift=0, lr_uv_shift=0,
                   lr_units=(None, None, None), reduced_tx_set=0, disable_cdf_update=0, tile_cols_log2=-1, tile_rows_log2=-1, opstream=False,
-                  visible=None, key_rows32=0, **arrays):
+                  visible=None, key_rows32=0, trace_tile=None, **arrays):
     f = ObuFrame()
     f.width, f.height, f.bit_depth, f.frame_type, f.base_q_idx = width, height, bit_depth, frame_type, base_q_idx
     if visible is not None:
@@ -75,6 +75,8 @@
     err = C.create_string_buffer(256)
     if opstream:
         h = lib()
+        if trace_tile is not None:
+            return _tile_trace(h, f, int(key_rows32), int(trace_tile))
         h.av1mi_host_opstream_key32_temporal_unit.restype = C.c_longlong
         h.av1mi_host_opstream_key32_temporal_unit.argtypes = [C.POINTER(ObuFrame), C.c_int, C.c_int, C.c_void_p, C.c_longlong, C.c_char_p, C.c_int]
         n = h.av1mi_host_opstream_key32_temporal_unit(C.byref(f), int(key_rows32), int(with_sequence_header), out.ctypes.data, cap, err, 256)
@@ -85,6 +87,22 @@
     if n > cap:
         raise RuntimeError("temporal unit of %d bytes exceeds the buffer" % n)
     return out[:n].tobytes()
+
+
+def _tile_trace(h, f, key_rows32, tile):
+    fn = h.av1mi_host_opstream_tile_trace
+    fn.restype = C.c_longlong
+    fn.argtypes = [C.POINTER(ObuFrame), C.c_int, C.c_int, C.c_void_p, C.c_void_p, C.c_void_p, C.c_longlong, C.c_void_p, C.c_int, C.c_void_p, C.c_int, C.c_void_p]
+    cap, slot_cap, image_cap = 1 << 17, 512, 1 << 14
+    lst, sym, con = (np.zeros(cap, np.uint32) for _ in range(3))
+    slots, image, counts = np.zeros((slot_cap, 4), np.uint16), np.zeros(image_cap, np.uint16), np.zeros(5, np.int64)
+    rc = fn(C.byref(f), key_rows32, tile, lst.ctypes.data, sym.ctypes.data, con.ctypes.data, cap, slots.ctypes.data, slot_cap, image.ctypes.data, image_cap,
+            counts.ctypes.data)
+    if rc < 0:
+        raise ValueError("op-stream tile trace failed (%d)" % rc)
+    nl, ng, ns, ni, nt = (int(v) for v in counts)
+    assert nl <= cap and ng <= cap and ns <= slot_cap and ni <= image_cap
+    return dict(list=lst[:nl], symbols=sym[:ng], consumed=con[:nl], slots=slots[:ns].astype(np.int64), image=image[:ni], ntiles=nt)
 
 
 BLOCK_DTYPE = np.dtype([("mi_row", "<u2"), ("mi_col", "<u2"), ("bsize", "u1"), ("skip", "u1"), ("is_inter", "u1"), ("y_mode", "u1"), ("uv_mode", "u1"),
diff --git a/av1-go_amd/csrc/av1_entropy_kernels.hip b/av1-go_amd/csrc/av1_entropy_kernels.hip
--- a/av1-go_amd/csrc/av1_entropy_kernels.hip
+++ b/av1-go_amd/csrc/av1_entropy_kernels.hip
@@ -207,9 +207,7 @@
 }
 
 __global__ __launch_bounds__(64) void k_av1_chains(Av1EntLaunch L, int ntiles_all, int ngroups) {
-  const int xcd = blockIdx.x & 7, j = blockIdx.x >> 3, nslots = L.nslots;
-  const int g = (j / nslots) * 8 + xcd, sl = j - (j / nslots) * nslots, lane = threadIdx.x, t = g * 64 + lane;
-  if (g >= ngroups) return;
+  const int nslots = L.nslots, g = blockIdx.x / nslots, sl = blockIdx.x - g * nslots, lane = threadIdx.x, t = g * 64 + lane;
   __shared__ __attribute__((aligned(16))) uint16_t s_big[64 * 16];
   const int n = L.tab.nsym[sl], off = L.tab.off[sl];
   int cnt = 0, base = 0;
@@ -217,20 +215,19 @@
   if (mine && L.band) { const int tiles = L.sbr_n * L.sbc_n, sbr = (t % tiles) / L.sbc_n; mine = (sbr < L.sb_rows32) == (L.band == 1); }
   if (mine) { cnt = L.slot_total[(size_t)t * S_MAX + sl]; base = L.slot_base[(size_t)t * S_MAX + sl]; }
   if (!__any(cnt > 0)) return;
-  const size_t tt = t < ntiles_all ? (size_t)t : 0;
-  op_t *list = L.ops + tt * L.ops_cap;
-  const uint32_t *grouped = L.grouped + tt * L.grouped_cap + base;
+  uint4 *g4 = reinterpret_cast<uint4 *>(L.grouped + (t < ntiles_all ? (size_t)t : 0) * L.grouped_cap + base);
+  const uint4 z = make_uint4(0, 0, 0, 0);
   if (n <= 4) {
     const uint32_t *iw = reinterpret_cast<const uint32_t *>(L.cdf_image) + (off >> 1);
     uint64_t cdf = (uint64_t)iw[0] | ((uint64_t)iw[1] << 32);
-    const uint4 *g4 = reinterpret_cast<const uint4 *>(grouped);
-    const uint4 z = make_uint4(0, 0, 0, 0);
     uint4 c0 = cnt > 0 ? g4[0] : z, c1 = cnt > 4 ? g4[1] : z, c2 = cnt > 8 ? g4[2] : z, c3 = cnt > 12 ? g4[3] : z;
-    auto four = [&](const uint4 &v, int e) {
-      if (e < cnt) list[v.x >> 4] = small_step(cdf, (int)(v.x & 15), n);
-      if (e + 1 < cnt) list[v.y >> 4] = small_step(cdf, (int)(v.y & 15), n);
-      if (e + 2 < cnt) list[v.z >> 4] = small_step(cdf, (int)(v.z & 15), n);
-      if (e + 3 < cnt) list[v.w >> 4] = small_step(cdf, (int)(v.w & 15), n);
+    auto four = [&](uint4 v, int e) {
+      if (e >= cnt) return;
+      v.x = small_step(cdf, (int)(v.x & 15), n);
+      if (e + 1 < cnt) v.y = small_step(cdf, (int)(v.y & 15), n);
+      if (e + 2 < cnt) v.z = small_step(cdf, (int)(v.z & 15), n);
+      if (e + 3 < cnt) v.w = small_step(cdf, (int)(v.w & 15), n);
+      g4[e >> 2] = v;
     };
 #pragma unroll 1
     for (int e = 0; e < cnt; e += 16) {
@@ -247,11 +244,17 @@
       d[0] = iw[0];
       d[1] = n > 8 ? iw[1] : make_uint4(0, 0, 0, 0);
     }
+    auto step = [&](uint32_t v) { const int s = (int)(v & 15); return (uint32_t)(s >= kSplitHorz ? split_tuple(cdf, s) : big_step(cdf, s, n)); };
+    uint4 c = cnt > 0 ? g4[0] : z;
 #pragma unroll 1
-    for (int e = 0; e < cnt; e++) {
-      const uint32_t v = grouped[e];
-      const int s = (int)(v & 15);
-      list[v >> 4] = s >= kSplitHorz ? split_tuple(cdf, s) : big_step(cdf, s, n);
+    for (int e = 0; e < cnt; e += 4) {
+      const uint4 nx = e + 4 < cnt ? g4[(e >> 2) + 1] : z;
+      c.x = step(c.x);
+      if (e + 1 < cnt) c.y = step(c.y);
+      if (e + 2 < cnt) c.z = step(c.z);
+      if (e + 3 < cnt) c.w = step(c.w);
+      g4[e >> 2] = c;
+      c = nx;
     }
   }
 }
@@ -267,35 +270,46 @@
   c.init(L.slots + (size_t)(live ? t : 0) * L.slot_cap, (int)L.slot_cap, s_lane + lane * kLaneWords + kRingOps * 2);
   const int n = live ? (int)L.nops[t] : 0;
   const uint4 *ops4 = reinterpret_cast<const uint4 *>(L.ops + (size_t)(live ? t : 0) * L.ops_cap);
-  uint4 r0, r1, r2, r3, r4, r5, r6, r7;
-  r0 = r1 = r2 = r3 = r4 = r5 = r6 = r7 = make_uint4(0, 0, 0, 0);
+  const uint32_t *grouped = L.grouped + (size_t)(live ? t : 0) * L.grouped_cap;
+  const uint32_t last_entry = L.grouped_cap - 1;
+  uint4 raw[8];
+  uint32_t res[32];
+#pragma unroll
+  for (int k = 0; k < 8; k++) raw[k] = make_uint4(0, 0, 0, 0);
+#pragma unroll
+  for (int k = 0; k < 32; k++) res[k] = 0;
   int w = 0;
-  bool pend = false;
-  auto request = [&]() {
-    const uint4 *p = ops4 + (w >> 2);
-    if (w < n) r0 = p[0];
-    if (w + 4 < n) r1 = p[1];
-    if (w + 8 < n) r2 = p[2];
-    if (w + 12 < n) r3 = p[3];
-    if (w + 16 < n) r4 = p[4];
-    if (w + 20 < n) r5 = p[5];
-    if (w + 24 < n) r6 = p[6];
-    if (w + 28 < n) r7 = p[7];
-    pend = w < n;
+  auto request = [&](int from) {
+    const uint4 *p = ops4 + (from >> 2);
+#pragma unroll
+    for (int k = 0; k < 8; k++) if (from + 4 * k < n) raw[k] = p[k];
+  };
+  auto resolve = [&](int from) {
+#pragma unroll
+    for (int k = 0; k < 8; k++) {
+      const uint32_t a[4] = { raw[k].x, raw[k].y, raw[k].z, raw[k].w };
+#pragma unroll
+      for (int q = 0; q < 4; q++) {
+        uint32_t v = a[q];
+        if (from + 4 * k + q < n && is_ref(v)) v = grouped[min(v & 0xFFFFu, last_entry)];
+        res[4 * k + q] = v;
+      }
+    }
   };
   auto take = [&]() {
-    uint4 *q = reinterpret_cast<uint4 *>(ring + (w & 32));
-    q[0] = r0; q[1] = r1; q[2] = r2; q[3] = r3; q[4] = r4; q[5] = r5; q[6] = r6; q[7] = r7;
+    uint4 *q = reinterpret_cast<uint4 *>(ring + (w & (kRingOps - 1)));
+#pragma unroll
+    for (int k = 0; k < 8; k++) q[k] = make_uint4(res[4 * k], res[4 * k + 1], res[4 * k + 2], res[4 * k + 3]);
     w += 32;
   };
-  request();
-  if (pend) { take(); request(); }
+  request(0); resolve(0); request(32);
+  take(); resolve(32); request(64);
   int i = 0, lit_left = 0;
   uint32_t op = ring[0], op_next = ring[1], op_next2 = ring[2];
   for (;;) {
     if (!__any(lit_left > 0 || i < n)) break;
-    if (__any((pend && w - i < 24) || c.ns >= Coder::kStage - 8)) {
-      if (pend && w - i <= 32) { take(); request(); }
+    if (__any((w < n && w - i < 24) || c.ns >= Coder::kStage - 8)) {
+      if (w < n && w - i <= kRingOps - 32) { take(); resolve(w); request(w + 32); }
       c.spill();
     }
 #pragma unroll
@@ -367,10 +381,10 @@
   t = ctx_prof_begin(ctx, AV1MI_K_ENTROPY_CHAINS, s);
   Av1EntLaunch C = L;
   C.nslots = L.fv.key ? S_KEY_END : S_INTER_END; C.band = L.sb_rows32 ? 2 : 0;
-  if (L.sb_rows32 < L.sbr_n) hipLaunchKernelGGL(k_av1_chains, dim3((unsigned)(((ngroups + 7) / 8) * 8 * C.nslots)), dim3(64), 0, s, C, ntiles_all, ngroups);
+  if (L.sb_rows32 < L.sbr_n) hipLaunchKernelGGL(k_av1_chains, dim3((unsigned)(ngroups * C.nslots)), dim3(64), 0, s, C, ntiles_all, ngroups);
   if (L.sb_rows32) {
     C.nslots = K_END; C.band = 1; C.tab = L.tab32; C.cdf_image = L.cdf_image32;
-    hipLaunchKernelGGL(k_av1_chains, dim3((unsigned)(((ngroups + 7) / 8) * 8 * C.nslots)), dim3(64), 0, s, C, ntiles_all, ngroups);
+    hipLaunchKernelGGL(k_av1_chains, dim3((unsigned)(ngroups * C.nslots)), dim3(64), 0, s, C, ntiles_all, ngroups);
   }
   ctx_prof_end(ctx, t, s);
   return hipGetLastError();
@@ -390,8 +404,8 @@
 }
 
 struct av1mi_av1ent_state {
-  void *info = nullptr, *ops[2] = { nullptr, nullptr }, *nops[2] = { nullptr, nullptr }, *grouped = nullptr, *slot_tb = nullptr, *rec = nullptr, *slots = nullptr, *tile_off = nullptr, *status = nullptr;
-  size_t info_b = 0, ops_b[2] = { 0, 0 }, nops_b[2] = { 0, 0 }, grouped_b = 0, slot_tb_b = 0, rec_b = 0, slots_b = 0, off_b = 0;
+  void *info = nullptr, *ops[2] = { nullptr, nullptr }, *nops[2] = { nullptr, nullptr }, *grouped[2] = { nullptr, nullptr }, *slot_tb = nullptr, *rec = nullptr, *slots = nullptr, *tile_off = nullptr, *status = nullptr;
+  size_t info_b = 0, ops_b[2] = { 0, 0 }, nops_b[2] = { 0, 0 }, grouped_b[2] = { 0, 0 }, slot_tb_b = 0, rec_b = 0, slots_b = 0, off_b = 0;
   hipEvent_t lists_ready[2] = { nullptr, nullptr }, lists_free[2] = { nullptr, nullptr };
   bool free_recorded[2] = { false, false };
   unsigned long jobs = 0;
@@ -478,12 +492,12 @@
   int rc;
   if ((rc = grow(ctx, &st->info, &st->info_b, nb * sizeof(av1ops::BlockInfo))) ||
       (rc = grow(ctx, &st->ops[par], &st->ops_b[par], nt * L.ops_cap * sizeof(av1ops::op_t))) || (rc = grow(ctx, &st->nops[par], &st->nops_b[par], nt * 4)) ||
-      (rc = grow(ctx, &st->grouped, &st->grouped_b, nt * L.grouped_cap * sizeof(uint32_t))) ||
+      (rc = grow(ctx, &st->grouped[par], &st->grouped_b[par], nt * L.grouped_cap * sizeof(uint32_t))) ||
       (rc = grow(ctx, &st->slot_tb, &st->slot_tb_b, nt * av1ops::S_MAX * 4)) ||
       (rc = grow(ctx, &st->rec, &st->rec_b, nt * av1ops::kBlocksPerTile * av1ops::kBlockRecords * sizeof(uint16_t))) ||
       (rc = grow(ctx, &st->slots, &st->slots_b, nt * L.slot_cap)) || (rc = grow(ctx, &st->tile_off, &st->off_b, (nt + 1) * 8)))
     return rc;
-  L.info = (av1ops::BlockInfo *)st->info; L.ops = (av1ops::op_t *)st->ops[par]; L.nops = (uint32_t *)st->nops[par]; L.grouped = (uint32_t *)st->grouped;
+  L.info = (av1ops::BlockInfo *)st->info; L.ops = (av1ops::op_t *)st->ops[par]; L.nops = (uint32_t *)st->nops[par]; L.grouped = (uint32_t *)st->grouped[par];
   L.slot_total = (uint16_t *)st->slot_tb; L.slot_base = L.slot_total + nt * av1ops::S_MAX; L.rec = (uint16_t *)st->rec; L.slots = (uint8_t *)st->slots;
   L.tile_off = (uint64_t *)st->tile_off;
   L.tile_size = j->d_tile_size; L.out = j->d_out; L.out_cap = j->out_cap;
@@ -550,7 +564,7 @@
 namespace av1mi {
 void av1ent_free(av1mi_av1ent_state *st) {
   if (!st) return;
-  for (void *p : { st->info, st->ops[0], st->ops[1], st->nops[0], st->nops[1], st->grouped, st->slot_tb, st->rec, st->slots, st->tile_off }) if (p) (void)hipFree(p);
+  for (void *p : { st->info, st->ops[0], st->ops[1], st->nops[0], st->nops[1], st->grouped[0], st->grouped[1], st->slot_tb, st->rec, st->slots, st->tile_off }) if (p) (void)hipFree(p);
   for (hipEvent_t ev : { st->lists_ready[0], st->lists_ready[1], st->lists_free[0], st->lists_free[1] }) if (ev) (void)hipEventDestroy(ev);
   for (auto &k : st->d_image) for (uint16_t *p : k) if (p) (void)hipFree(p);
   for (uint16_t *p : st->d_image32) if (p) (void)hipFree(p);
diff --git a/av1-go_amd/csrc/av1_ops.hpp b/av1-go_amd/csrc/av1_ops.hpp
--- a/av1-go_amd/csrc/av1_ops.hpp
+++ b/av1-go_amd/csrc/av1_ops.hpp
@@ -98,6 +98,9 @@
 typedef uint32_t op_t;
 struct SlotTable { uint16_t off[S_MAX]; uint8_t nsym[(S_MAX + 3) & ~3]; int words; };
 AV1_HD op_t op_lit(int n, unsigned v) { return (op_t)(0x80000000u | ((unsigned)n << 27) | (v & 0x7FFu)); }
+enum : uint32_t { kOpRef = 0x40000000u };
+AV1_HD op_t op_ref(unsigned pos) { return (op_t)(kOpRef | (pos & 0xFFFFu)); }
+AV1_HD bool is_ref(op_t e) { return (e & 0xC0000000u) == kOpRef; }
 AV1_HD op_t make_tuple(uint32_t fl, uint32_t fh, int s, int n) { return (op_t)(((unsigned)(n - s) << 19) | ((fl >> 6) << 9) | (fh >> 6)); }
 enum { kBlocksPerTile = 64, kSplitHorz = 14, kSplitVert = 15, kListAlign = 4, kBlockRecords = 1024 };
 
@@ -136,7 +139,7 @@
       if (r & 0x8000u) { if (literals) list[n] = op_lit((int)((r >> 11) & 15), r & 0x7FFu); }
       else {
         const int sl = (int)(r >> 4);
-        if (sl >= slot_lo && sl < slot_hi) { uint16_t &p = pos[(sl - slot_lo) * kBlocks + blk]; grouped[p] = ((uint32_t)n << 4) | (r & 15u); p++; }
+        if (sl >= slot_lo && sl < slot_hi) { uint16_t &p = pos[(sl - slot_lo) * kBlocks + blk]; grouped[p] = r & 15u; list[n] = op_ref(p); p++; }
       }
     }
   }
@@ -648,19 +651,21 @@
   return make_tuple(kind == kSplitHorz ? p2 + p3 + p4 + p6 + p7 + p9 : p1 + p3 + p4 + p5 + p6 + p8, 0, 1, 2);
 }
 
-AV1_HD void run_chain(const uint16_t *init, int n, const uint32_t *g, int cnt, op_t *list) {
+AV1_HD void run_chain(const uint16_t *init, int n, uint32_t *g, int cnt) {
   if (n <= 4) {
     uint64_t w = (uint64_t)init[0] | ((uint64_t)init[1] << 16) | ((uint64_t)init[2] << 32) | ((uint64_t)init[3] << 48);
-    for (int k = 0; k < cnt; k++) list[g[k] >> 4] = small_step(w, (int)(g[k] & 15), n);
+    for (int k = 0; k < cnt; k++) g[k] = small_step(w, (int)(g[k] & 15), n);
     return;
   }
   alignas(16) uint16_t v[16];
   for (int i = 0; i < 16; i++) v[i] = i < slot_words(n) ? init[i] : 0;
   for (int k = 0; k < cnt; k++) {
     const int s = (int)(g[k] & 15);
-    list[g[k] >> 4] = s >= kSplitHorz ? split_tuple(v, s) : big_step(v, s, n);
-  }
-}
+    g[k] = s >= kSplitHorz ? split_tuple(v, s) : big_step(v, s, n);
+  }
+}
+
+AV1_HD op_t resolve_word(op_t e, const uint32_t *grouped) { return is_ref(e) ? (op_t)grouped[e & 0xFFFFu] : e; }
 
 AV1_HD void code_word(Coder &c, op_t e) {
   if (e >> 31) { for (int i = (int)((e >> 27) & 15) - 1; i >= 0; i--) { c.bit((e >> i) & 1); if (c.stage_full()) c.spill(); } }
diff --git a/av1-go_amd/host/av1_bitstream.hpp b/av1-go_amd/host/av1_bitstream.hpp
--- a/av1-go_amd/host/av1_bitstream.hpp
+++ b/av1-go_amd/host/av1_bitstream.hpp
@@ -27,7 +27,14 @@
                           std::string *err);
 std::vector<uint8_t> range_code_raw(const uint32_t *fl, const uint32_t *fh, const uint8_t *sym, const uint8_t *nsym, size_t count);
 bool opstream_supported(const av1mi_obu_frame &f, std::string *why);
-bool opstream_tiles(const av1mi_obu_frame &f, std::vector<std::vector<uint8_t>> *tiles, std::string *err, int key_rows32 = 0);
+struct OpstreamTileTrace {
+  std::vector<uint32_t> list, symbols, consumed;
+  struct SlotUse { uint16_t base, total, off, nsym; };
+  std::vector<SlotUse> slots;
+  std::vector<uint16_t> image;
+};
+bool opstream_tiles(const av1mi_obu_frame &f, std::vector<std::vector<uint8_t>> *tiles, std::string *err, int key_rows32 = 0,
+                    std::vector<OpstreamTileTrace> *trace = nullptr);
 bool blocks_temporal_unit(const av1mi_obu_blocks &d, bool with_sequence_header, std::vector<uint8_t> *out, std::string *err, int threads = 1,
                           const size_t (*tile_start)[2] = nullptr);
 bool temporal_unit(const av1mi_obu_frame &f, bool with_sequence_header, int threads, std::vector<uint8_t> *out, std::string *err);
diff --git a/av1-go_amd/host/av1_opstream.cpp b/av1-go_amd/host/av1_opstream.cpp
--- a/av1-go_amd/host/av1_opstream.cpp
+++ b/av1-go_amd/host/av1_opstream.cpp
@@ -24,20 +24,30 @@
 namespace {
 template <int kBlocks>
 bool code_tile(const uint16_t *rec, int block_records, const int *nrec, const int *first, uint16_t *pos, int nslots, const uint16_t *total,
-               const uint16_t *base, int run, const av1ops::SlotTable &tab, const uint16_t *image, std::vector<uint8_t> *out, std::string *err) {
+               const uint16_t *base, int run, const av1ops::SlotTable &tab, const uint16_t *image, std::vector<uint8_t> *out, std::string *err,
+               OpstreamTileTrace *trace) {
   using namespace av1ops;
   if (run > 65535) { if (err) *err = "tile too large for 16-bit entry positions"; return false; }
   const int nops = first[kBlocks];
   std::vector<op_t> list((size_t)nops, 0);
   std::vector<uint32_t> grouped((size_t)run, 0);
   for (int b = 0; b < kBlocks; b++) replay_block<kBlocks>(rec + (size_t)b * block_records, nrec[b], pos, b, first[b], list.data(), grouped.data());
+  if (trace) {
+    trace->list = list; trace->symbols = grouped; trace->image.assign(image, image + tab.words); trace->consumed.clear();
+    trace->slots.clear();
+    for (int sl = 0; sl < nslots; sl++) trace->slots.push_back({ base[sl], total[sl], tab.off[sl], tab.nsym[sl] });
+  }
   for (int sl = 0; sl < nslots; sl++)
-    if (total[sl]) run_chain(&image[tab.off[sl]], tab.nsym[sl], &grouped[(size_t)base[sl]], total[sl], list.data());
+    if (total[sl]) run_chain(&image[tab.off[sl]], tab.nsym[sl], &grouped[(size_t)base[sl]], total[sl]);
   out->resize((size_t)nops * 2 + 64);
   Coder c;
   uint16_t stage[Coder::kStage];
   c.init(out->data(), (int)out->size(), stage);
-  for (int i = 0; i < nops; i++) code_word(c, list[(size_t)i]);
+  for (int i = 0; i < nops; i++) {
+    const op_t e = resolve_word(list[(size_t)i], grouped.data());
+    if (trace) trace->consumed.push_back(e);
+    code_word(c, e);
+  }
   const int n = c.finish();
   if (n < 0) { if (err) *err = "tile payload overflow"; return false; }
   out->resize((size_t)n);
@@ -45,7 +55,8 @@
 }
 }
 
-bool opstream_tiles(const av1mi_obu_frame &f, std::vector<std::vector<uint8_t>> *tiles, std::string *err, int key_rows32) {
+bool opstream_tiles(const av1mi_obu_frame &f, std::vector<std::vector<uint8_t>> *tiles, std::string *err, int key_rows32,
+                    std::vector<OpstreamTileTrace> *trace) {
   using namespace av1ops;
   if (!opstream_supported(f, err)) return false;
   if (key_rows32 && (f.frame_type != 0 || (key_rows32 & 63) || key_rows32 > f.height || (f.width & 31))) { if (err) *err = "bad 32x32 band"; return false; }
@@ -78,6 +89,7 @@
   const std::vector<uint16_t> image = default_slot_image(v.key != 0, qcat, &tab);
   const int sbr_n = (v.h8 + 7) / 8, sbc_n = (v.w8 + 7) / 8;
   tiles->assign((size_t)sbr_n * sbc_n, {});
+  if (trace) trace->assign((size_t)sbr_n * sbc_n, {});
   const int nslots = v.key ? S_KEY_END : S_INTER_END;
   std::vector<uint8_t> cnt((size_t)S_MAX * kBlocksPerTile);
   std::vector<uint16_t> pos((size_t)S_MAX * kBlocksPerTile), rec((size_t)kBlocksPerTile * kBlockRecords);
@@ -114,7 +126,7 @@
         uint16_t base[K_END], total[K_END];
         const int run = place_tile32(cnt32.data(), total, base);
         if (!code_tile<kBlocks32>(rec32.data(), kBlockRecords32, nrec, first, cnt32.data(), K_END, total, base, run, tab32, image32.data(),
-                                  &(*tiles)[(size_t)sbr * sbc_n + sbc], err))
+                                  &(*tiles)[(size_t)sbr * sbc_n + sbc], err, trace ? &(*trace)[(size_t)sbr * sbc_n + sbc] : nullptr))
           return false;
         continue;
       }
@@ -145,7 +157,7 @@
         run = (run + n + kListAlign - 1) & ~(kListAlign - 1);
       }
       if (!code_tile<kBlocksPerTile>(rec.data(), kBlockRecords, nrec, first, pos.data(), nslots, total, base, run, tab, image.data(),
-                                     &(*tiles)[(size_t)sbr * sbc_n + sbc], err))
+                                     &(*tiles)[(size_t)sbr * sbc_n + sbc], err, trace ? &(*trace)[(size_t)sbr * sbc_n + sbc] : nullptr))
         return false;
     }
   if (stats)
diff --git a/av1-go_amd/host/capi_host.cpp b/av1-go_amd/host/capi_host.cpp
--- a/av1-go_amd/host/capi_host.cpp
+++ b/av1-go_amd/host/capi_host.cpp
@@ -169,6 +169,19 @@
   if ((long long)b.size() <= cap && out) memcpy(out, b.data(), b.size());
   return (long long)b.size();
 }
+long long av1mi_host_opstream_tile_trace(const av1mi_obu_frame *f, int key_rows32, int tile, uint32_t *list, uint32_t *symbols, uint32_t *consumed,
+                                         long long cap_words, uint16_t *slots, int slot_cap, uint16_t *image, int image_cap, long long *counts) {
+  std::vector<std::vector<uint8_t>> tiles; std::vector<av1::OpstreamTileTrace> trace; std::string e;
+  if (!av1::opstream_supported(*f, &e)) return -2;
+  if (!av1::opstream_tiles(*f, &tiles, &e, key_rows32, &trace) || tile < 0 || (size_t)tile >= trace.size()) return -1;
+  const av1::OpstreamTileTrace &t = trace[(size_t)tile];
+  auto copy = [&](const std::vector<uint32_t> &v, uint32_t *dst) { if (dst) memcpy(dst, v.data(), std::min<size_t>(v.size(), (size_t)std::max(cap_words, 0LL)) * 4); };
+  copy(t.list, list); copy(t.symbols, symbols); copy(t.consumed, consumed);
+  for (size_t i = 0; slots && i < t.slots.size() && (int)i < slot_cap; i++) { slots[4 * i] = t.slots[i].base; slots[4 * i + 1] = t.slots[i].total; slots[4 * i + 2] = t.slots[i].off; slots[4 * i + 3] = t.slots[i].nsym; }
+  if (image) memcpy(image, t.image.data(), std::min<size_t>(t.image.size(), (size_t)std::max(image_cap, 0)) * 2);
+  if (counts) { counts[0] = (long long)t.list.size(); counts[1] = (long long)t.symbols.size(); counts[2] = (long long)t.slots.size(); counts[3] = (long long)t.image.size(); counts[4] = (long long)trace.size(); }
+  return 0;
+}
 long long av1mi_host_opstream_temporal_unit(const av1mi_obu_frame *f, int with_sequence_header, uint8_t *out, long long cap, char *err, int errcap) {
   return av1mi_host_opstream_key32_temporal_unit(f, 0, with_sequence_header, out, cap, err, errcap);
 }
```

Result: slower. 2393 (-15.0%).
